# david-cortes/cmfrec

Measured on AMD Instinct MI355X. Metric: ALS rows/sec ((users+items)/iteration time), implicit ALS-CG k=50 fp64, higher is better.
Workload: dtype f64

## Files before the change

cmfrec_amd/csrc/cg_kernels.hpp:

```cpp
#pragma once
#include <hip/hip_runtime.h>
#include <stdint.h>
#include <type_traits>

#include "lanes.hpp"

namespace cmfhip {

constexpr int WAVE = 64;
constexpr int TILE = 64;
constexpr int MAX_W = 8;
#ifndef CMF_CG_WAVES_PER_SIMD
#define CMF_CG_WAVES_PER_SIMD 2
#endif
#ifndef CMF_CG_WAVES_PER_SIMD_F32
#define CMF_CG_WAVES_PER_SIMD_F32 3
#endif
#ifndef CMF_CG_WAVES_PER_SIMD_LOW
#define CMF_CG_WAVES_PER_SIMD_LOW 3
#endif
constexpr int CG_NTSEL_MAX_S = 7;
template <typename T, int W, int NRES_, int NTSEL = 0> constexpr int cg_waves_per_simd()
{
    if (sizeof(T) == 8 && NTSEL == 1 && W <= 8) return CMF_CG_WAVES_PER_SIMD_LOW;
    if (sizeof(T) == 4 && NTSEL == 1 && W <= 4 && NRES_ == 0) return CMF_CG_WAVES_PER_SIMD_F32 + 1;
    return (sizeof(T) == 4 && W <= 4 && NRES_ == 0) ? CMF_CG_WAVES_PER_SIMD_F32 : CMF_CG_WAVES_PER_SIMD;
}
constexpr int CG_NT_LOW = 6;
#ifndef CMF_CG_NT_F32
#define CMF_CG_NT_F32 1
#endif
#ifndef CMF_CG_NT_MIN_S
#define CMF_CG_NT_MIN_S 4
#endif

struct RowDesc {
    int row;
    int nnz;
    unsigned long long st;
};

constexpr int CG_NCOUNTERS = 64;
constexpr int CG_COUNTER_STRIDE = 32;

template <typename T>
__device__ __forceinline__ T cg_div(T num, T den)
{
#ifndef CMF_CG_IEEE_DIV
    if constexpr (sizeof(T) == 4) return num * __builtin_amdgcn_rcpf(den);
    else {
        double y = __builtin_amdgcn_rcp(den);
        double e = __builtin_fma(-den, y, 1.0);
        y = __builtin_fma(y, e, y);
        e = __builtin_fma(-den, y, 1.0);
        y = __builtin_fma(y, e, y);
        double q = num * y;
        const double r = __builtin_fma(-den, q, num);
        return __builtin_fma(r, y, q);
    }
#else
    return num / den;
#endif
}

template <typename V>
__device__ __forceinline__ V lds_g(const V *p) { return *p; }

template <typename T>
struct CgParams {
    T *A;
    size_t lda;
    const T *B;
    size_t ldb;
    int k;
    const size_t *indptr;
    const int *indices;
    const T *values;
    const T *bias_sub;
    const T *weights = nullptr;
    const T *wsum = nullptr;
    const int *order;
    const RowDesc *desc;
    int nrows;
    const T *BtB;
    T lam, lam_last;
    int scale_lam, scale_bias_const;
    int max_cg_steps;
    int precond;
    int koff = 0, kc = 0;
    const T *CtC = nullptr;
    const T *UC = nullptr;
    T w_side = 0;
    int rows_with_u = 0;
    int row_first = 0;
    const size_t *indptr2 = nullptr;
    const int *indices2 = nullptr;
    const T *values2 = nullptr;
    const T *C2 = nullptr;
    int *counter = nullptr;
    int p_side = 0, scale_lam_sideinfo = 0;
    const T *Bi = nullptr;
    const T *BiTBi = nullptr;
    int ki = 0;
    T w_imp = 0;
    const T *rconst = nullptr;
    size_t ldr = 0;
    int gx = 0;
#ifdef CMF_CG_DEBUG
    int dbg = 0;
#endif
#ifdef CMF_CG_TICKS
    unsigned long long *ticks = nullptr;
#endif
};
#ifdef CMF_CG_TICKS
#define CMF_TICK() __builtin_amdgcn_s_memtime()
__device__ __forceinline__ void cg_ticks_flush(unsigned long long *t, int slot, unsigned long long wait, unsigned long long pass, unsigned long long rows,
                                               unsigned long long total, int lane)
{
    if (t != nullptr && lane == 0) {
        atomicAdd(t + 4 * slot + 0, wait); atomicAdd(t + 4 * slot + 1, pass); atomicAdd(t + 4 * slot + 2, rows); atomicAdd(t + 4 * slot + 3, total);
    }
}
#endif
#ifdef CMF_CG_DEBUG
#define CMF_DBG(P, bit) (((P).dbg & (bit)) != 0)
#else
#define CMF_DBG(P, bit) false
#endif
template <int NT, int S, typename TILE, typename T>
__device__ __forceinline__ void dbg_fill_tile(TILE &tile, T val)
{
#pragma unroll
    for (int t = 0; t < NT; t++)
#pragma unroll
        for (int s = 0; s < S; s++) tile.set(t, s, val);
}

template <typename T>
__device__ __forceinline__ T wave_sum(T v) { return lanes::wave_sum(v); }

template <typename T, int NT, int I>
__device__ __forceinline__ T treduce8_low_first(const T (&v)[8], bool h)
{
    if constexpr (I + 4 < NT) {
        T keep = h ? v[I + 4] : v[I];
        return keep + lanes::recv_xor4(v[I], v[I + 4]);
    } else return v[I] + lanes::xor4_lower(v[I]);
}
template <typename T, int NT = 8>
__device__ __forceinline__ T treduce8_low(const T (&v)[8], int lane)
{
    static_assert(NT >= 4 && NT <= 8, "entries per lane group");
    T u[4], q[2];
    bool h = (lane & 4) != 0;
    u[0] = treduce8_low_first<T, NT, 0>(v, h); u[1] = treduce8_low_first<T, NT, 1>(v, h);
    u[2] = treduce8_low_first<T, NT, 2>(v, h); u[3] = treduce8_low_first<T, NT, 3>(v, h);
    h = (lane & 2) != 0;
#pragma unroll
    for (int i = 0; i < 2; i++) {
        T keep = h ? u[i + 2] : u[i];
        T send = h ? u[i] : u[i + 2];
        q[i] = keep + lanes::xor2(send);
    }
    h = (lane & 1) != 0;
    T keep = h ? q[1] : q[0];
    T send = h ? q[0] : q[1];
    return keep + lanes::xor1(send);
}

template <typename T>
__device__ __forceinline__ T treduce8_high(const T (&v)[8], int lane)
{
    T u[4], q[2];
#pragma unroll
    for (int i = 0; i < 4; i++) u[i] = lanes::tswap32_add(v[i], v[i + 4]);
#pragma unroll
    for (int i = 0; i < 2; i++) q[i] = lanes::tswap16_add(u[i], u[i + 2]);
    const bool h = (lane & 8) != 0;
    T keep = h ? q[1] : q[0];
    return keep + lanes::recv_xor8(q[0], q[1]);
}

#ifndef CMF_PASS_VECTOR_LDS
#define CMF_PASS_VECTOR_LDS 2
#endif
template <typename T> constexpr bool pass_vector_in_lds() { return CMF_PASS_VECTOR_LDS == 1 || (CMF_PASS_VECTOR_LDS == 2 && sizeof(T) == 8); }
template <typename T, int S>
__device__ __forceinline__ void replicate(T vdist, T (&vrep)[S], int lane);
template <typename T, int S, int GR = 8>
__device__ __forceinline__ void pass_vector_lds(T vdist, T (&vrep)[S], T (&wts)[8], int lane, T *__restrict__ pv)
{
    const int jj = lane >> 3, ll = lane & 7;
    pv[lane] = vdist;
    __builtin_amdgcn_wave_barrier();
#pragma unroll
    for (int s = 0; s < S; s++) vrep[s] = pv[ll + 8 * s];
    const T *wp = pv + GR * jj;
#pragma unroll
    for (int t = 0; t < GR; t++) wts[t] = wp[t];
    __builtin_amdgcn_wave_barrier();
}

__host__ __device__ constexpr int gram_ld(int S) { return 8 * S + 1; }
#ifndef CMF_GRAM_ROWS_BY_K
#define CMF_GRAM_ROWS_BY_K 1
#endif
template <typename T> __host__ __device__ constexpr int gram_rows(int S) { return (CMF_GRAM_ROWS_BY_K && pass_vector_in_lds<T>()) ? S : 8; }
__host__ __device__ constexpr int gram_ld_rows(int S, int GR)
{
    if (GR == 8) return gram_ld(S);
    int ld = 8 * S;
    while ((S * ld) % 32 != 8 && (S * ld) % 32 != 24) ld++;
    return ld;
}
__host__ __device__ constexpr int gram_ld2(int S) { return 8 * S + 2; }
template <typename T> __host__ __device__ constexpr int gram_elems(int S) { return sizeof(T) == 4 ? 64 * gram_ld2(S) : 64 * gram_ld(S); }
template <typename T, int S, int GR = 8> __device__ __forceinline__ int gram_index(int r, int c)
{
    if constexpr (sizeof(T) == 4) return 2 * ((r >> 1) * gram_ld2(S) + c) + (r & 1);
    else return r * gram_ld_rows(S, GR) + c;
}
template <typename T, int S, int GR = 8>
__device__ __forceinline__ void stage_gramian(T *__restrict__ G, const T *__restrict__ BtB, int k, int tid, int nthreads)
{
    static_assert(GR == 8 || sizeof(T) == 8, "rows by k: double precision");
    for (int e = tid; e < 8 * GR * 8 * S; e += nthreads) {
        const int r = e / (8 * S), c = e % (8 * S);
        G[gram_index<T, S, GR>(r, c)] = (r < k && c < k) ? BtB[(size_t)r * k + c] : T(0);
    }
}

template <typename T, int S>
struct RegTile {
    T v[8][S];
    __device__ __forceinline__ void set(int t, int s, T x) { v[t][s] = x; }
};
typedef float f32x2 __attribute__((ext_vector_type(2)));
template <int S>
struct RegTile<float, S> {
    f32x2 v[4][S];
    __device__ __forceinline__ void set(int t, int s, float x) { v[t >> 1][s][t & 1] = x; }
};

template <typename T>
struct PassAcc {
    T v[8];
    __device__ __forceinline__ void zero()
    {
#pragma unroll
        for (int s = 0; s < 8; s++) v[s] = T(0);
    }
    __device__ __forceinline__ void close(T (&out)[8]) const
    {
#pragma unroll
        for (int s = 0; s < 8; s++) out[s] = v[s];
    }
};
template <>
struct PassAcc<float> {
    f32x2 v[8];
    __device__ __forceinline__ void zero()
    {
#pragma unroll
        for (int s = 0; s < 8; s++) v[s] = f32x2{0.f, 0.f};
    }
    __device__ __forceinline__ void close(float (&out)[8]) const
    {
#pragma unroll
        for (int s = 0; s < 8; s++) out[s] = v[s][0] + v[s][1];
    }
};

template <typename T, int S, int NT = 8>
__device__ __forceinline__ void load_tile(RegTile<T, S> &tile, const T *__restrict__ Bm, size_t ldb,
                                          int k, int my_idx, int cnt, int lane)
{
    const int jj = lane >> 3, ll = lane & 7;
    int its[8];
    its[0] = lanes::bcast8<0>(my_idx); its[1] = lanes::bcast8<1>(my_idx); its[2] = lanes::bcast8<2>(my_idx);
    its[3] = lanes::bcast8<3>(my_idx);
    if (NT > 4) its[4] = lanes::bcast8<4>(my_idx);
    if (NT > 5) its[5] = lanes::bcast8<5>(my_idx);
    if (NT > 6) its[6] = lanes::bcast8<6>(my_idx);
    if (NT > 7) its[7] = lanes::bcast8<7>(my_idx);
    const int first_idx = __builtin_amdgcn_readfirstlane(my_idx);
    const int col_last = min(ll + 8 * (S - 1), k - 1) - ll;
    const char *base = reinterpret_cast<const char *>(Bm + ll);
    const unsigned ldb_bytes = (unsigned)(ldb * sizeof(T));
#pragma unroll
    for (int t = 0; t < NT; t++) {
        const unsigned it = (unsigned)(((jj * NT + t) < cnt) ? its[t] : first_idx);
        const T *rp = reinterpret_cast<const T *>(base + (unsigned long long)it * ldb_bytes);
#pragma unroll
        for (int s = 0; s < S; s++) tile.set(t, s, rp[(s < S - 1) ? 8 * s : col_last]);
    }
}

template <typename T, bool IMPLICIT, int MODE>
__device__ __forceinline__ T pass_weight(T coef, T x, bool valid, T g = T(1))
{
    T w;
    if (IMPLICIT) {
        if (MODE == 0) w = -(coef - T(1)) * x - coef;
        else           w = coef * (x - T(1)) + coef;
    } else {
        if (MODE == 0) w = -((coef - x) * g);
        else           w = coef * g;
    }
    return valid ? w : T(0);
}

template <typename T>
__device__ __forceinline__ T row_lam_mult(const CgParams<T> &P, int row, int nnz)
{
    return (P.wsum != nullptr) ? P.wsum[row] : (T)nnz;
}
template <typename T, bool IMPLICIT>
__device__ __forceinline__ T entry_weight(const CgParams<T> &P, size_t pos)
{
    if (IMPLICIT) return T(1);
    return (P.weights != nullptr) ? P.weights[pos] : T(1);
}

template <int S, bool IMPLICIT, int MODE, int NT = 8, bool INIT = false>
__device__ __forceinline__ void tile_pass_f32(const RegTile<float, S> &tile, const float (&vrep)[S], float x, bool valid,
                                          PassAcc<float> &out, int lane, float g = 1.f)
{
    static_assert(NT % 2 == 0, "single precision: the entries of a lane group travel in pairs");
    float c[8];
#pragma unroll
    for (int q = 0; q < NT / 2; q++) {
        f32x2 acc = f32x2{0.f, 0.f};
#pragma unroll
        for (int s = 0; s < S; s++) acc += tile.v[q][s] * f32x2{vrep[s], vrep[s]};
        c[2 * q] = acc[0]; c[2 * q + 1] = acc[1];
    }
    float coef = treduce8_low<float, NT>(c, lane);
    const float w = pass_weight<float, IMPLICIT, MODE>(coef, x, valid, g);
    float wts[8];
    wts[0] = lanes::bcast8<0>(w); wts[1] = lanes::bcast8<1>(w); wts[2] = lanes::bcast8<2>(w); wts[3] = lanes::bcast8<3>(w);
    if (NT > 4) { wts[4] = lanes::bcast8<4>(w); wts[5] = lanes::bcast8<5>(w); }
    if (NT > 6) { wts[6] = lanes::bcast8<6>(w); wts[7] = lanes::bcast8<7>(w); }
#pragma unroll
    for (int q = 0; q < NT / 2; q++) {
        const f32x2 w2 = f32x2{wts[2 * q], wts[2 * q + 1]};
#pragma unroll
        for (int s = 0; s < S; s++) out.v[s] = (INIT && q == 0) ? w2 * tile.v[q][s] : out.v[s] + w2 * tile.v[q][s];
    }
    if constexpr (INIT) {
#pragma unroll
        for (int s = S; s < 8; s++) out.v[s] = f32x2{0.f, 0.f};
    }
}

template <typename T, int S, bool IMPLICIT, int MODE, int NT = 8, bool INIT = false>
__device__ __forceinline__ void tile_pass(const RegTile<T, S> &tile, const T (&vrep)[S], T x, bool valid,
                                          PassAcc<T> &out, int lane, T g = T(1))
{
    if constexpr (std::is_same<T, float>::value) {
        tile_pass_f32<S, IMPLICIT, MODE, NT, INIT>(tile, vrep, x, valid, out, lane, g);
    } else {
    T c[8];
#pragma unroll
    for (int t = 0; t < NT; t++) {
        T acc = T(0);
#pragma unroll
        for (int s = 0; s < S; s++) acc += tile.v[t][s] * vrep[s];
        c[t] = acc;
    }
    T coef = treduce8_low<T, NT>(c, lane);
    const T w = pass_weight<T, IMPLICIT, MODE>(coef, x, valid, g);
    T wts[8];
    wts[0] = lanes::bcast8<0>(w); wts[1] = lanes::bcast8<1>(w); wts[2] = lanes::bcast8<2>(w); wts[3] = lanes::bcast8<3>(w);
    if (NT > 4) wts[4] = lanes::bcast8<4>(w);
    if (NT > 5) wts[5] = lanes::bcast8<5>(w);
    if (NT > 6) wts[6] = lanes::bcast8<6>(w);
    if (NT > 7) wts[7] = lanes::bcast8<7>(w);
#pragma unroll
    for (int t = 0; t < NT; t++) {
#pragma unroll
        for (int s = 0; s < S; s++) out.v[s] = (INIT && t == 0) ? wts[t] * tile.v[t][s] : out.v[s] + wts[t] * tile.v[t][s];
    }
    if constexpr (INIT) {
#pragma unroll
        for (int s = S; s < 8; s++) out.v[s] = T(0);
    }
    }
}

template <typename T, int S, int W>
__device__ __forceinline__ void gram_pass(const T *__restrict__ G, T wdist, PassAcc<T> &out, int lane, int wr)
{
    constexpr int LD = gram_ld(S);
    const int jj = lane >> 3, ll = lane & 7;
    T wts[8];
    wts[0] = lanes::bcast8<0>(wdist); wts[1] = lanes::bcast8<1>(wdist); wts[2] = lanes::bcast8<2>(wdist);
    wts[3] = lanes::bcast8<3>(wdist); wts[4] = lanes::bcast8<4>(wdist); wts[5] = lanes::bcast8<5>(wdist);
    wts[6] = lanes::bcast8<6>(wdist); wts[7] = lanes::bcast8<7>(wdist);
    if constexpr (std::is_same<T, float>::value && W <= 4) {
#pragma unroll
        for (int q = 0; q < 4; q++) {
            if (W > 1 && (q % W) != wr) continue;
            const f32x2 *g = reinterpret_cast<const f32x2 *>(G) + (jj * 4 + q) * gram_ld2(S) + ll;
            const f32x2 w2 = f32x2{wts[2 * q], wts[2 * q + 1]};
#pragma unroll
            for (int s = 0; s < S; s++) out.v[s] += w2 * lds_g(g + 8 * s);
        }
    } else {
#pragma unroll
        for (int t = 0; t < 8; t++) {
            if (W > 1 && (t % W) != wr) continue;
#pragma unroll
            for (int s = 0; s < S; s++) {
                if constexpr (std::is_same<T, float>::value) out.v[s][0] += wts[t] * G[gram_index<T, S>(jj * 8 + t, ll + 8 * s)];
                else out.v[s] += wts[t] * lds_g(G + (jj * 8 + t) * LD + ll + 8 * s);
            }
        }
    }
}

template <bool NEG, typename T, int S, int W, int GR = 8>
__device__ __forceinline__ void gram_pass_w(const T *__restrict__ G, const T (&wts)[8], PassAcc<T> &out, int lane, int wr)
{
    constexpr int LD = gram_ld_rows(S, GR);
    const int jj = lane >> 3, ll = lane & 7;
    if constexpr (std::is_same<T, float>::value && W <= 4) {
#pragma unroll
        for (int q = 0; q < 4; q++) {
            if (W > 1 && (q % W) != wr) continue;
            const f32x2 *g = reinterpret_cast<const f32x2 *>(G) + (jj * 4 + q) * gram_ld2(S) + ll;
            const f32x2 w2 = f32x2{wts[2 * q], wts[2 * q + 1]};
#pragma unroll
            for (int s = 0; s < S; s++) out.v[s] = NEG ? out.v[s] - w2 * lds_g(g + 8 * s) : out.v[s] + w2 * lds_g(g + 8 * s);
        }
    } else {
#pragma unroll
        for (int t = 0; t < GR; t++) {
            if (W > 1 && (t % W) != wr) continue;
#pragma unroll
            for (int s = 0; s < S; s++) {
                if constexpr (std::is_same<T, float>::value) {
                    const float g = G[gram_index<T, S>(jj * 8 + t, ll + 8 * s)];
                    out.v[s][0] = NEG ? out.v[s][0] - wts[t] * g : out.v[s][0] + wts[t] * g;
                } else {
                    const T g = lds_g(G + (jj * GR + t) * LD + ll + 8 * s);
                    out.v[s] = NEG ? out.v[s] - wts[t] * g : out.v[s] + wts[t] * g;
                }
            }
        }
    }
}

template <typename T, int S>
__device__ __forceinline__ void replicate(T vdist, T (&vrep)[S], int lane)
{
    const int ll = lane & 7;
#pragma unroll
    for (int s = 0; s < S; s++) vrep[s] = __shfl(vdist, s * 8 + ll);
}

template <typename T, int S, bool IMPLICIT, int W, int RPB, bool GRAMX = false, int NRES_ = 0, int NTSEL = 0>
__global__ void __launch_bounds__(64 * W * RPB, (cg_waves_per_simd<T, W, NRES_, NTSEL>()))
cg_rows_kernel(const CgParams<T> P)
{
    constexpr bool GRAM = IMPLICIT || GRAMX;
    extern __shared__ __attribute__((aligned(16))) unsigned char smem_raw[];
    T *G = reinterpret_cast<T *>(smem_raw);
    T *red = G + (GRAM ? gram_elems<T>(S) : 0);
    const int tid = threadIdx.x;
    const int lane = tid & 63;
    const int wave = tid >> 6;
    const int grp = wave / W;
    const int wr = wave % W;
    const int k = P.k;

    const int nteams = gridDim.x * RPB;
    __shared__ int s_claim[4];
    constexpr bool PV = pass_vector_in_lds<T>();
    __shared__ __attribute__((aligned(16))) T s_pv[PV ? W * RPB : 1][PV ? 64 : 1];
    const int cslot = (blockIdx.x * RPB + grp) % CG_NCOUNTERS;
    int *const my_counter = P.counter + cslot * CG_COUNTER_STRIDE;
    const int cbase = nteams + cslot;
    auto issue_claim = [&]() -> int {
        int v = 0;
        if (wr == 0 && lane == 0) v = atomicAdd(my_counter, 1);
        return v;
    };
    int rnxt, rnn;
    if (W == 1) {
        const int c1 = issue_claim(), c2 = issue_claim();
        rnxt = cbase + CG_NCOUNTERS * __builtin_amdgcn_readfirstlane(c1);
        rnn = cbase + CG_NCOUNTERS * __builtin_amdgcn_readfirstlane(c2);
    } else if (wr == 0 && lane == 0) {
        s_claim[2] = cbase + CG_NCOUNTERS * atomicAdd(my_counter, 1);
        s_claim[3] = cbase + CG_NCOUNTERS * atomicAdd(my_counter, 1);
    }
    constexpr int GR = gram_rows<T>(S);
    if (GRAM) stage_gramian<T, S, GR>(G, P.BtB, k, tid, blockDim.x);
    if (GRAM || W > 1) __syncthreads();
    if (W > 1) { rnxt = s_claim[2]; rnn = s_claim[3]; }
    T *myred = red + (size_t)grp * 2 * W * 64;

    int buf = 0;
    static_assert(W == 1 || RPB == 1, "multi-wave teams own their workgroup (barriers are per row)");

    constexpr int NRES = NRES_ > 0 ? NRES_ : ((std::is_same<T, float>::value && W == 8) ? 2 : 1);
    static_assert(NRES == 1 || std::is_same<T, float>::value, "two resident tiles: single precision");
    static_assert(NTSEL == 0 || (S >= CMF_CG_NT_MIN_S && (sizeof(T) == 4 || S <= CG_NTSEL_MAX_S) && NRES_ == 0),
                  "launches by tile size: tiles by row length (double precision: k <= 56)");
    constexpr int NT_MIN = (S >= CMF_CG_NT_MIN_S && (CMF_CG_NT_F32 || !std::is_same<T, float>::value)) ? (std::is_same<T, float>::value ? 6 : 5) : 8;
    auto nt_of = [&](int nnz_) -> int {
        int nt = (nnz_ + 8 * W * NRES - 1) / (8 * W * NRES);
        if (std::is_same<T, float>::value) nt = (nt + 1) & ~1;
        return (nt > 8) ? 8 : (nt < NT_MIN ? NT_MIN : nt);
    };
    struct Pre { int idx; T x; T a; int idx2; T x2; T g; T g2; };
    auto load_desc = [&](int rix_) -> RowDesc {
        RowDesc d; d.row = 0; d.nnz = 0; d.st = 0;
        if (rix_ < P.nrows) d = P.desc[rix_];
        d.row = __builtin_amdgcn_readfirstlane(d.row);
        d.nnz = __builtin_amdgcn_readfirstlane(d.nnz);
        d.st = ((unsigned long long)(unsigned)__builtin_amdgcn_readfirstlane((int)(d.st >> 32)) << 32) |
               (unsigned)__builtin_amdgcn_readfirstlane((int)(d.st & 0xffffffffu));
        return d;
    };
    auto load_pre = [&](const RowDesc &d) -> Pre {
        Pre q; q.idx = 0; q.x = T(0); q.a = T(0); q.idx2 = 0; q.x2 = T(0); q.g = T(1); q.g2 = T(1);
        const int nt = nt_of(d.nnz), tl = 8 * nt;
        const int b = lane & 7;
        const int ent = (lane >> 3) * nt + b;
        const int cnt = min(tl, d.nnz - wr * tl);
        if (b < nt && ent < cnt) {
            const size_t pos = d.st + (size_t)wr * tl + ent;
            q.idx = P.indices[pos];
            q.x = P.values[pos];
            q.g = entry_weight<T, IMPLICIT>(P, pos);
            if (!IMPLICIT && P.bias_sub != nullptr) q.x -= P.bias_sub[q.idx];
        }
        if (NRES == 2) {
            const int cnt2 = min(tl, d.nnz - (wr + W) * tl);
            if (b < nt && ent < cnt2) {
                const size_t pos = d.st + (size_t)(wr + W) * tl + ent;
                q.idx2 = P.indices[pos];
                q.x2 = P.values[pos];
                q.g2 = entry_weight<T, IMPLICIT>(P, pos);
                if (!IMPLICIT && P.bias_sub != nullptr) q.x2 -= P.bias_sub[q.idx2];
            }
        }
        if (d.nnz > 0 && lane < k) q.a = P.A[(size_t)d.row * P.lda + lane];
        return q;
    };
    int rix = blockIdx.x * RPB + grp;
    RowDesc dcur = load_desc(rix);
    RowDesc dnxt = load_desc(rnxt);
    Pre pcur = load_pre(dcur);
    int pend = issue_claim();
#ifdef CMF_CG_TICKS
    unsigned long long tk_wait = 0, tk_pass = 0, tk_rows = 0;
    const unsigned long long tk_begin = CMF_TICK();
#endif
    int it = 0;
    RowDesc dnn;
    Pre pnxt;
    auto solve_row = [&](auto nt_tag) {
        constexpr int NT = decltype(nt_tag)::value;
        constexpr int TL = 8 * NT;
        const int row = dcur.row;
        const size_t st = dcur.st;
        const int nnz = dcur.nnz;
        const int ntiles = (nnz + TL - 1) / TL;
        const int my_ntiles = (ntiles > wr) ? (ntiles - wr + W - 1) / W : 0;
        const bool resident = NT < 8 || my_ntiles <= NRES;

        T lam = P.lam, lam_last = P.lam_last;
        if (GRAMX && P.kc > 0) {
            if (P.scale_lam || P.scale_lam_sideinfo) {
                T mult = row_lam_mult(P, row, nnz);
                if (P.scale_lam_sideinfo) mult += (T)P.p_side;
                lam *= mult; lam_last *= mult;
            }
        } else if (!IMPLICIT && P.scale_lam) {
            const T mult = row_lam_mult(P, row, nnz);
            lam *= mult;
            if (!P.scale_bias_const) lam_last *= mult;
        }
        T *arow = P.A + (size_t)row * P.lda;
        T a_d = pcur.a;

        RegTile<T, S> tile;
        const int ent = (lane >> 3) * NT + (lane & 7);
        const bool lane_has = (NT == 8) || (lane & 7) < NT;
        const int cnt0 = min(TL, nnz - wr * TL);
        T x_res = pcur.x;
        const T g_res = pcur.g;
        bool valid_res = lane_has && ent < cnt0;
        if (CMF_DBG(P, 1)) dbg_fill_tile<8, S>(tile, (T)(pcur.idx & 3) * (T)0.001);
        else if (cnt0 > 0) load_tile<T, S, NT>(tile, P.B, P.ldb, k, pcur.idx, cnt0, lane);
        RegTile<T, (NRES == 2) ? S : 1> tile2;
        const int cnt1 = (NRES == 2) ? min(TL, nnz - (wr + W) * TL) : 0;
        const T x2_res = pcur.x2, g2_res = pcur.g2;
        const bool valid2_res = lane_has && ent < cnt1;
        if constexpr (NRES == 2) {
            if (cnt1 > 0 && !CMF_DBG(P, 1)) load_tile<T, S, NT>(tile2, P.B, P.ldb, k, pcur.idx2, cnt1, lane);
        }
        dnn = load_desc(rnn);
        pnxt = load_pre(dnxt);
#ifdef CMF_CG_TICKS
        const unsigned long long tk0 = CMF_TICK();
        asm volatile("s_waitcnt vmcnt(0)" ::: "memory");
        const unsigned long long tk1 = CMF_TICK();
        tk_wait += tk1 - tk0;
#endif

        auto run_pass = [&](T vdist, auto mode_tag, bool first) -> T {
            constexpr int MODE = decltype(mode_tag)::value;
            asm volatile("" ::: "memory");
            T vrep[S];
            T gw[8];
            if constexpr (PV) pass_vector_lds<T, S, GR>(vdist, vrep, gw, lane, &s_pv[wave][0]);
            else replicate<T, S>(vdist, vrep, lane);
            PassAcc<T> acc;
            acc.zero();
            if constexpr (NRES == 2) {
                if (cnt0 > 0 && !CMF_DBG(P, 4)) tile_pass<T, S, IMPLICIT, MODE, NT>(tile, vrep, x_res, valid_res, acc, lane, g_res);
                if (cnt1 > 0 && !CMF_DBG(P, 4)) tile_pass<T, S, IMPLICIT, MODE, NT>(tile2, vrep, x2_res, valid2_res, acc, lane, g2_res);
            } else if constexpr (NT < 8) {
                if (cnt0 > 0 && !CMF_DBG(P, 4)) tile_pass<T, S, IMPLICIT, MODE, NT>(tile, vrep, x_res, valid_res, acc, lane, g_res);
            } else
            for (int tl = wr; tl < ntiles; tl += W) {
                T x, g; bool valid;
                const bool have = (tl == wr) && (resident || first);
                if (!have) {
                    const int cnt = min(TL, nnz - tl * TL);
                    valid = lane_has && ent < cnt;
                    const size_t pos = st + (size_t)tl * TL + ent;
                    int my_idx = valid ? P.indices[pos] : 0;
                    x = valid ? P.values[pos] : T(0);
                    g = valid ? entry_weight<T, IMPLICIT>(P, pos) : T(1);
                    if (!IMPLICIT && P.bias_sub != nullptr && valid) x -= P.bias_sub[my_idx];
                    if (!CMF_DBG(P, 1)) load_tile<T, S, NT>(tile, P.B, P.ldb, k, my_idx, cnt, lane);
                } else {
                    x = x_res; g = g_res; valid = valid_res;
                }
                if (!CMF_DBG(P, 4)) tile_pass<T, S, IMPLICIT, MODE, NT>(tile, vrep, x, valid, acc, lane, g);
            }
            if (GRAM && !CMF_DBG(P, 2)) {
                if constexpr (PV) gram_pass_w<MODE == 0, T, S, W, GR>(G, gw, acc, lane, wr);
                else gram_pass<T, S, W>(G, (MODE == 0) ? -vdist : vdist, acc, lane, wr);
            }
            T out[8];
            acc.close(out);
            T tot = treduce8_high<T>(out, lane);
            if (W > 1) {
                T *rb = myred + (size_t)buf * W * 64;
                rb[wr * 64 + lane] = tot;
                if (first && wr == 0 && lane == 0) s_claim[it & 1] = cbase + CG_NCOUNTERS * pend;
                __syncthreads();
                tot = T(0);
#pragma unroll
                for (int w = 0; w < W; w++) tot += rb[w * 64 + lane];
                buf ^= 1;
            }
            return tot;
        };

        T r_d = run_pass(a_d, std::integral_constant<int, 0>{}, true);
        r_d -= lam * a_d;
        if (!IMPLICIT && lam != lam_last && lane == k - 1) r_d -= (lam_last - lam) * a_d;
        if (GRAMX && P.rconst != nullptr && lane < k) r_d += P.rconst[(size_t)row * P.ldr + lane];
        if (lane >= k) r_d = T(0);
        T p_d = r_d;
        T r_old = CMF_DBG(P, 8) ? T(1) : wave_sum(r_d * r_d);
        bool done = (r_old <= (T)1e-12);
        for (int step = 0; step < P.max_cg_steps && !done; step++) {
            T Ap_d = run_pass(p_d, std::integral_constant<int, 1>{}, false);
            Ap_d += lam * p_d;
            if (!IMPLICIT && lam != lam_last && lane == k - 1) Ap_d += (lam_last - lam) * p_d;
            if (lane >= k) Ap_d = T(0);
            T alpha = CMF_DBG(P, 8) ? T(0.001) : cg_div(r_old, wave_sum(Ap_d * p_d));
            a_d += alpha * p_d;
            r_d -= alpha * Ap_d;
            T r_new = CMF_DBG(P, 8) ? T(0.5) : wave_sum(r_d * r_d);
            if (r_new <= (T)1e-8) done = true;
            else {
                p_d = p_d * cg_div(r_new, r_old) + r_d;
                r_old = r_new;
            }
        }
        if (wr == 0 && lane < k) arow[lane] = a_d;
#ifdef CMF_CG_TICKS
        tk_pass += CMF_TICK() - tk1; tk_rows += (wr == 0);
#endif
    };
    for (; rix < P.nrows; it++) {
        const int nt = nt_of(dcur.nnz);
        if constexpr (NT_MIN == 8) solve_row(std::integral_constant<int, 8>{});
        else if constexpr (std::is_same<T, float>::value) {
            if constexpr (NTSEL == 1) solve_row(std::integral_constant<int, 6>{});
            else if constexpr (NTSEL == 2) solve_row(std::integral_constant<int, 8>{});
            else if (nt == 6) solve_row(std::integral_constant<int, 6>{});
            else solve_row(std::integral_constant<int, 8>{});
        } else if constexpr (NTSEL == 1) {
            if (nt <= 5) solve_row(std::integral_constant<int, 5>{});
            else solve_row(std::integral_constant<int, 6>{});
        } else if constexpr (NTSEL == 2) {
            if (nt <= 7) solve_row(std::integral_constant<int, 7>{});
            else solve_row(std::integral_constant<int, 8>{});
        } else {
            switch (nt) {
                case 5: solve_row(std::integral_constant<int, 5>{}); break;
                case 6: solve_row(std::integral_constant<int, 6>{}); break;
                case 7: solve_row(std::integral_constant<int, 7>{}); break;
                default: solve_row(std::integral_constant<int, 8>{}); break;
            }
        }
        const int r3 = (W == 1) ? cbase + CG_NCOUNTERS * __builtin_amdgcn_readfirstlane(pend) : s_claim[it & 1];
        dcur = dnxt; dnxt = dnn; pcur = pnxt;
        rix = rnxt; rnxt = rnn; rnn = r3;
        pend = issue_claim();
    }
#ifdef CMF_CG_TICKS
    cg_ticks_flush(P.ticks, W == 1 ? 0 : W == 2 ? 1 : W == 4 ? 2 : 3, tk_wait, tk_pass, tk_rows, CMF_TICK() - tk_begin, lane);
#endif
}

constexpr int TILE4 = 32;

template <typename T, int S>
struct RegTile4 {
    T v[4][S];
    __device__ __forceinline__ void set(int t, int s, T x) { v[t][s] = x; }
    __device__ __forceinline__ T get(int t, int s) const { return v[t][s]; }
};
template <int S>
struct RegTile4<float, S> {
    f32x2 v[2][S];
    __device__ __forceinline__ void set(int t, int s, float x) { v[t >> 1][s][t & 1] = x; }
    __device__ __forceinline__ f32x2 pair0(int s) const { return v[0][s]; }
};

template <typename T, int S>
__device__ __forceinline__ void load_tile4(RegTile4<T, S> &tile, const T *__restrict__ Bm, size_t ldb,
                                           int k, int my_idx, int cnt, int lane)
{
    const int jj = lane >> 3, ll = lane & 7;
    int its[4];
    its[0] = lanes::bcast8<0>(my_idx); its[1] = lanes::bcast8<2>(my_idx);
    its[2] = lanes::bcast8<4>(my_idx); its[3] = lanes::bcast8<6>(my_idx);
    const int first_idx = __builtin_amdgcn_readfirstlane(my_idx);
    const int col_last = min(ll + 8 * (S - 1), k - 1) - ll;
    const char *base = reinterpret_cast<const char *>(Bm + ll);
    const unsigned ldb_bytes = (unsigned)(ldb * sizeof(T));
#pragma unroll
    for (int t = 0; t < 4; t++) {
        const unsigned it = (unsigned)(((jj * 4 + t) < cnt) ? its[t] : first_idx);
        const T *rp = reinterpret_cast<const T *>(base + (unsigned long long)it * ldb_bytes);
#pragma unroll
        for (int s = 0; s < S; s++) tile.set(t, s, rp[(s < S - 1) ? 8 * s : col_last]);
    }
}

template <typename T>
__device__ __forceinline__ T treduce4_low(const T (&v)[4], int lane)
{
    T u[2];
    bool h = (lane & 4) != 0;
#pragma unroll
    for (int i = 0; i < 2; i++) {
        T keep = h ? v[i + 2] : v[i];
        u[i] = keep + lanes::recv_xor4(v[i], v[i + 2]);
    }
    h = (lane & 2) != 0;
    T keep = h ? u[1] : u[0];
    T send = h ? u[0] : u[1];
    T q = keep + lanes::xor2(send);
    return q + lanes::xor1(q);
}

template <int S, bool IMPLICIT, int MODE, typename TILE, bool INIT = false>
__device__ __forceinline__ void tile_pass4_f32(const TILE &tile, const float (&vrep)[S], float x, bool valid,
                                           PassAcc<float> &out, int lane, float g = 1.f)
{
    float c[4];
#pragma unroll
    for (int q = 0; q < 2; q++) {
        f32x2 acc = f32x2{0.f, 0.f};
#pragma unroll
        for (int s = 0; s < S; s++) acc += tile.v[q][s] * f32x2{vrep[s], vrep[s]};
        c[2 * q] = acc[0]; c[2 * q + 1] = acc[1];
    }
    float coef = treduce4_low<float>(c, lane);
    const float w = pass_weight<float, IMPLICIT, MODE>(coef, x, valid, g);
    float wts[4];
    wts[0] = lanes::bcast8<0>(w); wts[1] = lanes::bcast8<2>(w); wts[2] = lanes::bcast8<4>(w); wts[3] = lanes::bcast8<6>(w);
#pragma unroll
    for (int q = 0; q < 2; q++) {
        const f32x2 w2 = f32x2{wts[2 * q], wts[2 * q + 1]};
#pragma unroll
        for (int s = 0; s < S; s++) out.v[s] = (INIT && q == 0) ? w2 * tile.v[q][s] : out.v[s] + w2 * tile.v[q][s];
    }
    if constexpr (INIT) {
#pragma unroll
        for (int s = S; s < 8; s++) out.v[s] = f32x2{0.f, 0.f};
    }
}

template <typename T, int S, bool IMPLICIT, int MODE, typename TILE, bool INIT = false>
__device__ __forceinline__ void tile_pass4(const TILE &tile, const T (&vrep)[S], T x, bool valid,
                                           PassAcc<T> &out, int lane, T g = T(1))
{
    if constexpr (std::is_same<T, float>::value) {
        tile_pass4_f32<S, IMPLICIT, MODE, TILE, INIT>(tile, vrep, x, valid, out, lane, g);
    } else {
    T c[4];
#pragma unroll
    for (int t = 0; t < 4; t++) {
        T acc = T(0);
#pragma unroll
        for (int s = 0; s < S; s++) acc += tile.v[t][s] * vrep[s];
        c[t] = acc;
    }
    T coef = treduce4_low<T>(c, lane);
    const T w = pass_weight<T, IMPLICIT, MODE>(coef, x, valid, g);
    T wts[4];
    wts[0] = lanes::bcast8<0>(w); wts[1] = lanes::bcast8<2>(w); wts[2] = lanes::bcast8<4>(w); wts[3] = lanes::bcast8<6>(w);
#pragma unroll
    for (int t = 0; t < 4; t++) {
#pragma unroll
        for (int s = 0; s < S; s++) out.v[s] = (INIT && t == 0) ? wts[t] * tile.v[t][s] : out.v[s] + wts[t] * tile.v[t][s];
    }
    if constexpr (INIT) {
#pragma unroll
        for (int s = S; s < 8; s++) out.v[s] = T(0);
    }
    }
}

template <typename T, int S>
struct RegTile2 {
    T v[2][S];
    __device__ __forceinline__ void set(int t, int s, T x) { v[t][s] = x; }
    __device__ __forceinline__ T get(int t, int s) const { return v[t][s]; }
};
template <int S>
struct RegTile2<float, S> {
    f32x2 v[S];
    __device__ __forceinline__ void set(int t, int s, float x) { v[s][t] = x; }
    __device__ __forceinline__ f32x2 pair0(int s) const { return v[s]; }
};

template <typename T, int S, typename TILE>
__device__ __forceinline__ void load_tile2(TILE &tile, const T *__restrict__ Bm, size_t ldb,
                                           int k, int my_idx, int cnt, int lane)
{
    const int jj = lane >> 3, ll = lane & 7;
    int its[2];
    its[0] = lanes::bcast8<0>(my_idx); its[1] = lanes::bcast8<4>(my_idx);
    const int first_idx = __builtin_amdgcn_readfirstlane(my_idx);
    const int col_last = min(ll + 8 * (S - 1), k - 1) - ll;
    const char *base = reinterpret_cast<const char *>(Bm + ll);
    const unsigned ldb_bytes = (unsigned)(ldb * sizeof(T));
#pragma unroll
    for (int t = 0; t < 2; t++) {
        const unsigned it = (unsigned)(((jj * 2 + t) < cnt) ? its[t] : first_idx);
        const T *rp = reinterpret_cast<const T *>(base + (unsigned long long)it * ldb_bytes);
#pragma unroll
        for (int s = 0; s < S; s++) tile.set(t, s, rp[(s < S - 1) ? 8 * s : col_last]);
    }
}

template <typename T>
__device__ __forceinline__ T treduce2_low(const T (&v)[2], int lane)
{
    const bool h = (lane & 4) != 0;
    T u = (h ? v[1] : v[0]) + lanes::recv_xor4(v[0], v[1]);
    u += lanes::xor2(u);
    return u + lanes::xor1(u);
}

template <typename T, int S, bool IMPLICIT, int MODE, typename TILE, bool INIT = false>
__device__ __forceinline__ void tile_pass2(const TILE &tile, const T (&vrep)[S], T x, bool valid,
                                           PassAcc<T> &out, int lane, T g = T(1))
{
    T c[2];
    if constexpr (std::is_same<T, float>::value) {
        f32x2 acc = f32x2{0.f, 0.f};
#pragma unroll
        for (int s = 0; s < S; s++) acc += tile.pair0(s) * f32x2{vrep[s], vrep[s]};
        c[0] = acc[0]; c[1] = acc[1];
    } else {
#pragma unroll
        for (int t = 0; t < 2; t++) {
            T acc = T(0);
#pragma unroll
            for (int s = 0; s < S; s++) acc += tile.get(t, s) * vrep[s];
            c[t] = acc;
        }
    }
    const T coef = treduce2_low<T>(c, lane);
    const T w = pass_weight<T, IMPLICIT, MODE>(coef, x, valid, g);
    const T w0 = lanes::bcast8<0>(w), w1 = lanes::bcast8<4>(w);
    if constexpr (std::is_same<T, float>::value) {
        const f32x2 w2 = f32x2{w0, w1};
#pragma unroll
        for (int s = 0; s < S; s++) out.v[s] = INIT ? w2 * tile.pair0(s) : out.v[s] + w2 * tile.pair0(s);
        if constexpr (INIT) {
#pragma unroll
            for (int s = S; s < 8; s++) out.v[s] = f32x2{0.f, 0.f};
        }
    } else {
#pragma unroll
        for (int s = 0; s < S; s++) out.v[s] = INIT ? w0 * tile.get(0, s) : out.v[s] + w0 * tile.get(0, s);
#pragma unroll
        for (int s = 0; s < S; s++) out.v[s] += w1 * tile.get(1, s);
        if constexpr (INIT) {
#pragma unroll
            for (int s = S; s < 8; s++) out.v[s] = T(0);
        }
    }
}

template <typename T, int S, int NE> struct TinyTile { using type = RegTile4<T, S>; };
template <typename T, int S> struct TinyTile<T, S, 2> { using type = RegTile2<T, S>; };

#ifndef CMF_TINY_WAVES_PER_SIMD
#define CMF_TINY_WAVES_PER_SIMD 4
#endif
#ifndef CMF_TINY_GREG_F32
#define CMF_TINY_GREG_F32 1
#endif
#ifndef CMF_TINY_GREG_F64
#define CMF_TINY_GREG_F64 1
#endif
template <typename T, bool GRAM> constexpr bool tiny_greg() { return GRAM && (sizeof(T) == 8 ? CMF_TINY_GREG_F64 != 0 : CMF_TINY_GREG_F32 != 0); }
template <typename T, bool GRAM> constexpr int tiny_waves_per_simd() { return tiny_greg<T, GRAM>() ? (sizeof(T) == 8 ? 2 : 3) : CMF_TINY_WAVES_PER_SIMD; }
template <typename T, int S, int GR = 8>
struct GramRegs {
    T v[GR][S];
    __device__ __forceinline__ void load(const T *__restrict__ G, int lane)
    {
        const int jj = lane >> 3, ll = lane & 7;
#pragma unroll
        for (int t = 0; t < GR; t++)
#pragma unroll
            for (int s = 0; s < S; s++) v[t][s] = G[gram_index<T, S, GR>(jj * GR + t, ll + 8 * s)];
    }
};
template <int S>
struct GramRegs<float, S, 8> {
    f32x2 v[4][S];
    __device__ __forceinline__ void load(const float *__restrict__ G, int lane)
    {
        const int jj = lane >> 3, ll = lane & 7;
#pragma unroll
        for (int q = 0; q < 4; q++) {
            const f32x2 *g = reinterpret_cast<const f32x2 *>(G) + (jj * 4 + q) * gram_ld2(S) + ll;
#pragma unroll
            for (int s = 0; s < S; s++) v[q][s] = g[8 * s];
        }
    }
};
template <int S>
__device__ __forceinline__ void gram_pass_regs(const GramRegs<float, S> &R, float wdist, PassAcc<float> &out)
{
    float wts[8];
    wts[0] = lanes::bcast8<0>(wdist); wts[1] = lanes::bcast8<1>(wdist); wts[2] = lanes::bcast8<2>(wdist);
    wts[3] = lanes::bcast8<3>(wdist); wts[4] = lanes::bcast8<4>(wdist); wts[5] = lanes::bcast8<5>(wdist);
    wts[6] = lanes::bcast8<6>(wdist); wts[7] = lanes::bcast8<7>(wdist);
#pragma unroll
    for (int q = 0; q < 4; q++) {
        const f32x2 w2 = f32x2{wts[2 * q], wts[2 * q + 1]};
#pragma unroll
        for (int s = 0; s < S; s++) out.v[s] += w2 * R.v[q][s];
    }
}
template <typename T, int S>
__device__ __forceinline__ void gram_pass_regs(const GramRegs<T, S> &R, T wdist, PassAcc<T> &out)
{
    T wts[8];
    wts[0] = lanes::bcast8<0>(wdist); wts[1] = lanes::bcast8<1>(wdist); wts[2] = lanes::bcast8<2>(wdist);
    wts[3] = lanes::bcast8<3>(wdist); wts[4] = lanes::bcast8<4>(wdist); wts[5] = lanes::bcast8<5>(wdist);
    wts[6] = lanes::bcast8<6>(wdist); wts[7] = lanes::bcast8<7>(wdist);
#pragma unroll
    for (int t = 0; t < 8; t++)
#pragma unroll
        for (int s = 0; s < S; s++) out.v[s] += wts[t] * R.v[t][s];
}

template <bool NEG, int S>
__device__ __forceinline__ void gram_pass_regs_w(const GramRegs<float, S> &R, const float (&wts)[8], PassAcc<float> &out)
{
#pragma unroll
    for (int q = 0; q < 4; q++) {
        const f32x2 w2 = f32x2{wts[2 * q], wts[2 * q + 1]};
#pragma unroll
        for (int s = 0; s < S; s++) out.v[s] = NEG ? out.v[s] - w2 * R.v[q][s] : out.v[s] + w2 * R.v[q][s];
    }
}
template <bool NEG, typename T, int S, int GR>
__device__ __forceinline__ void gram_pass_regs_w(const GramRegs<T, S, GR> &R, const T (&wts)[8], PassAcc<T> &out)
{
#pragma unroll
    for (int t = 0; t < GR; t++)
#pragma unroll
        for (int s = 0; s < S; s++) out.v[s] = NEG ? out.v[s] - wts[t] * R.v[t][s] : out.v[s] + wts[t] * R.v[t][s];
}

template <typename T, int S, bool IMPLICIT, bool GRAMX = false, int NE = 4>
__global__ void __launch_bounds__(256, (tiny_waves_per_simd<T, IMPLICIT || GRAMX>()))
cg_rows_tiny_kernel(const CgParams<T> P)
{
    static_assert(NE == 4 || NE == 2 || NE == 0, "entries per lane group");
    constexpr bool MIX = NE == 0;
    static_assert(!MIX || CMF_TINY_WAVES_PER_SIMD >= 3, "the mixed launch lives in the dynamically scheduled loop");
    using Tile = typename TinyTile<T, S, (NE == 2) ? 2 : 4>::type;
    constexpr bool GRAM = IMPLICIT || GRAMX;
    extern __shared__ __attribute__((aligned(16))) unsigned char smem_raw[];
    T *G = reinterpret_cast<T *>(smem_raw);
    constexpr bool PV = pass_vector_in_lds<T>();
    __shared__ __attribute__((aligned(16))) T s_pv[PV ? 4 : 1][PV ? 64 : 1];
    const int tid = threadIdx.x;
    const int lane = tid & 63;
    auto short_row = [&](int nnz_) -> bool { return MIX && nnz_ <= 16; };
    auto entry_of = [&](int nnz_) -> int { return (NE == 2 || short_row(nnz_)) ? (lane >> 2) : (lane >> 1); };
    const int k = P.k;
    constexpr bool GREG = tiny_greg<T, GRAM>();
    constexpr int GR = GREG ? gram_rows<T>(S) : 8;
    if (GRAM) {
        stage_gramian<T, S, GR>(G, P.BtB, k, tid, blockDim.x);
        __syncthreads();
    }
    GramRegs<T, GREG ? S : 1, GREG ? GR : 8> greg;
    if constexpr (GREG) greg.load(G, lane);
    const int nwaves = gridDim.x * 4;
    struct Pre { int idx; T x; T a; T g; };
    auto load_desc = [&](int rix_) -> RowDesc {
        RowDesc d; d.row = 0; d.nnz = 0; d.st = 0;
        if (rix_ < P.nrows) d = P.desc[rix_];
        d.row = __builtin_amdgcn_readfirstlane(d.row);
        d.nnz = __builtin_amdgcn_readfirstlane(d.nnz);
        d.st = ((unsigned long long)(unsigned)__builtin_amdgcn_readfirstlane((int)(d.st >> 32)) << 32) |
               (unsigned)__builtin_amdgcn_readfirstlane((int)(d.st & 0xffffffffu));
        return d;
    };
    auto load_pre = [&](const RowDesc &d) -> Pre {
        Pre q; q.idx = 0; q.x = T(0); q.a = T(0); q.g = T(1);
        const int ent = entry_of(d.nnz);
        if (ent < d.nnz) {
            const size_t pos = d.st + (size_t)ent;
            q.idx = P.indices[pos];
            q.x = P.values[pos];
            q.g = entry_weight<T, IMPLICIT>(P, pos);
            if (!IMPLICIT && P.bias_sub != nullptr) q.x -= P.bias_sub[q.idx];
        }
        if (d.nnz > 0 && lane < k) q.a = P.A[(size_t)d.row * P.lda + lane];
        return q;
    };
    auto load_tile_ne = [&](Tile &t_, const T *Bm_, size_t ldb_, int k_, int idx_, int cnt_, int lane_) {
        if constexpr (NE != 2) load_tile4<T, S>(t_, Bm_, ldb_, k_, idx_, cnt_, lane_);
        else load_tile2<T, S>(t_, Bm_, ldb_, k_, idx_, cnt_, lane_);
    };
    auto solve = [&](const RowDesc &d, const Pre &pr, const Tile &tile, auto short_tag) {
        constexpr bool T2 = NE == 2 || decltype(short_tag)::value;
        const int nnz = d.nnz;
        T lam = P.lam, lam_last = P.lam_last;
        if (GRAMX && P.kc > 0) {
            if (P.scale_lam || P.scale_lam_sideinfo) {
                T mult = row_lam_mult(P, d.row, nnz);
                if (P.scale_lam_sideinfo) mult += (T)P.p_side;
                lam *= mult; lam_last *= mult;
            }
        } else if (!IMPLICIT && P.scale_lam) {
            const T mult = row_lam_mult(P, d.row, nnz);
            lam *= mult;
            if (!P.scale_bias_const) lam_last *= mult;
        }
        const bool valid = (T2 ? (lane >> 2) : (lane >> 1)) < nnz;
        T a_d = pr.a;
        auto run_pass = [&](T vdist, auto mode_tag) -> T {
            constexpr int MODE = decltype(mode_tag)::value;
            asm volatile("" ::: "memory");
            T vrep[S];
            T gw[8];
            if constexpr (PV) pass_vector_lds<T, S, GR>(vdist, vrep, gw, lane, &s_pv[tid >> 6][0]);
            else replicate<T, S>(vdist, vrep, lane);
            PassAcc<T> acc;
            if (!CMF_DBG(P, 4)) {
                if constexpr (!T2) tile_pass4<T, S, IMPLICIT, MODE, decltype(tile), true>(tile, vrep, pr.x, valid, acc, lane, pr.g);
                else tile_pass2<T, S, IMPLICIT, MODE, decltype(tile), true>(tile, vrep, pr.x, valid, acc, lane, pr.g);
            } else acc.zero();
            if constexpr (GREG) {
                if (!CMF_DBG(P, 2)) {
                    if constexpr (PV) gram_pass_regs_w<MODE == 0>(greg, gw, acc);
                    else gram_pass_regs(greg, (MODE == 0) ? -vdist : vdist, acc);
                }
            }
            else if (GRAM && !CMF_DBG(P, 2)) gram_pass<T, S, 1>(G, (MODE == 0) ? -vdist : vdist, acc, lane, 0);
            T out[8];
            acc.close(out);
            return treduce8_high<T>(out, lane);
        };
        T r_d = run_pass(a_d, std::integral_constant<int, 0>{});
        r_d -= lam * a_d;
        if (!IMPLICIT && lam != lam_last && lane == k - 1) r_d -= (lam_last - lam) * a_d;
        if (GRAMX && P.rconst != nullptr && lane < k) r_d += P.rconst[(size_t)d.row * P.ldr + lane];
        if (lane >= k) r_d = T(0);
        T p_d = r_d;
        T r_old = wave_sum(r_d * r_d);
        bool done = (r_old <= (T)1e-12);
        for (int step = 0; step < P.max_cg_steps && !done; step++) {
            T Ap_d = run_pass(p_d, std::integral_constant<int, 1>{});
            Ap_d += lam * p_d;
            if (!IMPLICIT && lam != lam_last && lane == k - 1) Ap_d += (lam_last - lam) * p_d;
            if (lane >= k) Ap_d = T(0);
            T alpha = cg_div(r_old, wave_sum(Ap_d * p_d));
            a_d += alpha * p_d;
            r_d -= alpha * Ap_d;
            T r_new = wave_sum(r_d * r_d);
            if (r_new <= (T)1e-8) done = true;
            else {
                p_d = p_d * cg_div(r_new, r_old) + r_d;
                r_old = r_new;
            }
        }
        if (lane < k) P.A[(size_t)d.row * P.lda + lane] = a_d;
    };

    int rix = blockIdx.x * 4 + (tid >> 6);
#if CMF_TINY_WAVES_PER_SIMD >= 3
    {
        const int cslot = rix % CG_NCOUNTERS;
        int *const my_counter = P.counter + cslot * CG_COUNTER_STRIDE;
        const int cbase = nwaves + cslot;
        auto issue_claim = [&]() -> int {
            int v = 0;
            if (lane == 0) v = atomicAdd(my_counter, 1);
            return v;
        };
        const int c1 = issue_claim(), c2 = issue_claim();
        int rnxt = cbase + CG_NCOUNTERS * __builtin_amdgcn_readfirstlane(c1);
        int rnn = cbase + CG_NCOUNTERS * __builtin_amdgcn_readfirstlane(c2);
        RowDesc d0 = load_desc(rix), d1 = load_desc(rnxt);
        Pre p0 = load_pre(d0);
        Tile tA;
        int pend = issue_claim();
        while (rix < P.nrows) {
            const bool shrt = short_row(d0.nnz);
            if (CMF_DBG(P, 1)) {
                dbg_fill_tile<(NE == 2) ? 2 : 4, S>(tA, (T)(p0.idx & 3) * (T)0.001);
            } else if constexpr (MIX) {
                if (shrt) load_tile2<T, S>(tA, P.B, P.ldb, k, p0.idx, d0.nnz, lane);
                else load_tile_ne(tA, P.B, P.ldb, k, p0.idx, d0.nnz, lane);
            } else load_tile_ne(tA, P.B, P.ldb, k, p0.idx, d0.nnz, lane);
            RowDesc d2 = load_desc(rnn);
            Pre p1 = load_pre(d1);
            if constexpr (MIX) {
                if (shrt) solve(d0, p0, tA, std::true_type{});
                else solve(d0, p0, tA, std::false_type{});
            } else solve(d0, p0, tA, std::false_type{});
            const int r3 = cbase + CG_NCOUNTERS * __builtin_amdgcn_readfirstlane(pend);
            d0 = d1; p0 = p1; d1 = d2;
            rix = rnxt; rnxt = rnn; rnn = r3;
            pend = issue_claim();
        }
        return;
    }
#endif
    RowDesc d0 = load_desc(rix), d1 = load_desc(rix + nwaves), d2 = load_desc(rix + 2 * nwaves);
    Pre p0 = load_pre(d0);
    Tile tA, tB;
    if (d0.nnz > 0) load_tile_ne(tA, P.B, P.ldb, k, p0.idx, d0.nnz, lane);
    Pre p1 = load_pre(d1);
    while (rix < P.nrows) {
        if (d1.nnz > 0) load_tile_ne(tB, P.B, P.ldb, k, p1.idx, d1.nnz, lane);
        RowDesc d3 = load_desc(rix + 3 * nwaves);
        Pre p2 = load_pre(d2);
        solve(d0, p0, tA, std::false_type{});
        rix += nwaves;
        if (rix >= P.nrows) break;
        if (d2.nnz > 0) load_tile_ne(tA, P.B, P.ldb, k, p2.idx, d2.nnz, lane);
        RowDesc d4 = load_desc(rix + 3 * nwaves);
        Pre p3 = load_pre(d3);
        solve(d1, p1, tB, std::false_type{});
        rix += nwaves;
        d0 = d2; p0 = p2; d1 = d3; p1 = p3; d2 = d4;
    }
}

constexpr int VH_CHUNK_TILES = 4;

struct VhWork {
    int vi;
    int row;
    int cnt;
    int chunk;
    unsigned long long st;
    unsigned long long pad_;
};

template <typename T>
struct VhState {
    T *r, *p;
    T *r_old;
    int *done;
    T *part;
    const int *chunk_row;
    const int *chunk_start;
    const int *chunk_cnt;
    const int *chunk_off;
    const int *launch;
    const VhWork *work;
    int nvh, nchunks, nlaunch;
};

template <typename T, int S, bool IMPLICIT, int MODE>
__global__ void __launch_bounds__(64 * VH_CHUNK_TILES, 3)
vh_pass_kernel(const CgParams<T> P, const VhState<T> V)
{
    __shared__ T red[VH_CHUNK_TILES][64];
    const int lane = threadIdx.x & 63, wave = threadIdx.x >> 6;
    const VhWork wk = V.work[blockIdx.x];
    const int vi = wk.vi;
    if (vi < 0) return;
    if (MODE == 1 && V.done[vi]) return;
    const int c = wk.chunk;
    const int row = wk.row;
    const size_t st = (size_t)wk.st;
    const int nnz = wk.cnt;
    const int tl = wave;
    const int k = P.k;
    T vdist;
    if (MODE == 0) vdist = (lane < k) ? P.A[(size_t)row * P.lda + lane] : T(0);
    else           vdist = V.p[(size_t)vi * 64 + lane];
    PassAcc<T> acc;
    acc.zero();
    if (tl * TILE < nnz) {
        const int cnt = min(TILE, nnz - tl * TILE);
        const bool valid = lane < cnt;
        const size_t pos = st + (size_t)tl * TILE + lane;
        int my_idx = valid ? P.indices[pos] : 0;
        T x = valid ? P.values[pos] : T(0);
        const T g = valid ? entry_weight<T, IMPLICIT>(P, pos) : T(1);
        if (!IMPLICIT && P.bias_sub != nullptr && valid) x -= P.bias_sub[my_idx];
        RegTile<T, S> tile;
        if (CMF_DBG(P, 1)) dbg_fill_tile<8, S>(tile, (T)(my_idx & 3) * (T)0.001);
        else load_tile<T, S>(tile, P.B, P.ldb, k, my_idx, cnt, lane);
        T vrep[S];
        replicate<T, S>(vdist, vrep, lane);
        if (!CMF_DBG(P, 4)) tile_pass<T, S, IMPLICIT, MODE>(tile, vrep, x, valid, acc, lane, g);
    }
    T out[8];
    acc.close(out);
    T tot = treduce8_high<T>(out, lane);
    red[wave][lane] = tot;
    __syncthreads();
    if (wave == 0) {
        T s = T(0);
#pragma unroll
        for (int w = 0; w < VH_CHUNK_TILES; w++) s += red[w][lane];
        V.part[(size_t)c * 64 + lane] = s;
    }
}

constexpr int VH_UPD_WAVES = 4;

template <typename T, bool IMPLICIT, int MODE, bool GRAMX = false>
__global__ void __launch_bounds__(64 * VH_UPD_WAVES)
vh_update_kernel(const CgParams<T> P, const VhState<T> V)
{
    __shared__ T psum[VH_UPD_WAVES][64];
    const int lane = threadIdx.x & 63, wave = threadIdx.x >> 6;
    const int vi = blockIdx.x;
    if (MODE == 1 && V.done[vi]) return;
    const int k = P.k;
    const int row = P.order[vi];
    const int nnz = (int)(P.indptr[row + 1] - P.indptr[row]);
    {
        const int c0 = V.chunk_off[vi], c1 = V.chunk_off[vi + 1];
        T acc = T(0);
        int c = c0 + wave;
        for (; c + 3 * VH_UPD_WAVES < c1; c += 4 * VH_UPD_WAVES) {
            T v0 = V.part[(size_t)c * 64 + lane];
            T v1 = V.part[(size_t)(c + VH_UPD_WAVES) * 64 + lane];
            T v2 = V.part[(size_t)(c + 2 * VH_UPD_WAVES) * 64 + lane];
            T v3 = V.part[(size_t)(c + 3 * VH_UPD_WAVES) * 64 + lane];
            acc += v0; acc += v1; acc += v2; acc += v3;
        }
        for (; c < c1; c += VH_UPD_WAVES) acc += V.part[(size_t)c * 64 + lane];
        psum[wave][lane] = acc;
    }
    __syncthreads();
    if (wave != 0) return;
    T tot = T(0);
#pragma unroll
    for (int w = 0; w < VH_UPD_WAVES; w++) tot += psum[w][lane];
    T lam = P.lam, lam_last = P.lam_last;
    if (GRAMX && P.kc > 0) {
        if (P.scale_lam || P.scale_lam_sideinfo) {
            T mult = row_lam_mult(P, row, nnz);
            if (P.scale_lam_sideinfo) mult += (T)P.p_side;
            lam *= mult; lam_last *= mult;
        }
    } else if (!IMPLICIT && P.scale_lam) {
        const T mult = row_lam_mult(P, row, nnz);
        lam *= mult;
        if (!P.scale_bias_const) lam_last *= mult;
    }
    T *arow = P.A + (size_t)row * P.lda;
    T a_d = (lane < k) ? arow[lane] : T(0);
    T v = (MODE == 0) ? a_d : V.p[(size_t)vi * 64 + lane];
    if (IMPLICIT || GRAMX) {
        T g = T(0);
        for (int j = 0; j < k; j++) {
            T vj = __shfl(v, j);
            if (lane < k) g += vj * P.BtB[(size_t)j * k + lane];
        }
        tot += (MODE == 0) ? -g : g;
    }
    if (MODE == 0) {
        T r_d = tot - lam * a_d;
        if (!IMPLICIT && lam != lam_last && lane == k - 1) r_d -= (lam_last - lam) * a_d;
        if (GRAMX && P.rconst != nullptr && lane < k) r_d += P.rconst[(size_t)row * P.ldr + lane];
        if (lane >= k) r_d = T(0);
        T r_old = wave_sum(r_d * r_d);
        V.r[(size_t)vi * 64 + lane] = r_d;
        V.p[(size_t)vi * 64 + lane] = r_d;
        if (lane == 0) { V.r_old[vi] = r_old; V.done[vi] = (r_old <= (T)1e-12) ? 1 : 0; }
    } else {
        T p_d = v;
        T r_d = V.r[(size_t)vi * 64 + lane];
        T r_old = V.r_old[vi];
        T Ap_d = tot + lam * p_d;
        if (!IMPLICIT && lam != lam_last && lane == k - 1) Ap_d += (lam_last - lam) * p_d;
        if (lane >= k) Ap_d = T(0);
        T alpha = cg_div(r_old, wave_sum(Ap_d * p_d));
        a_d += alpha * p_d;
        r_d -= alpha * Ap_d;
        T r_new = wave_sum(r_d * r_d);
        if (lane < k) arow[lane] = a_d;
        if (r_new <= (T)1e-8) {
            if (lane == 0) V.done[vi] = 1;
        } else {
            V.p[(size_t)vi * 64 + lane] = p_d * cg_div(r_new, r_old) + r_d;
            V.r[(size_t)vi * 64 + lane] = r_d;
            if (lane == 0) V.r_old[vi] = r_new;
        }
    }
}

template <typename T, int NF, bool IMPLICIT, int TEAM>
__global__ void __launch_bounds__(TEAM == 16 ? 1024 : 256)
cg_rows_generic_kernel(const CgParams<T> P)
{
    static_assert(TEAM == 1 || TEAM == 4 || TEAM == 16, "team");
    __shared__ T red[TEAM][64 * NF];
    const int lane = threadIdx.x & 63, wv = threadIdx.x >> 6;
    const int unit_global = (TEAM == 1) ? ((blockIdx.x * blockDim.x + threadIdx.x) >> 6) : (int)blockIdx.x;
    const int nunits = (TEAM == 1) ? ((gridDim.x * blockDim.x) >> 6) : (int)gridDim.x;
    const int kx = P.k, koff = P.koff, kt = koff + kx, kc = P.kc;
    const bool coll = kc > 0;
    for (int rix = P.row_first + unit_global; rix < P.nrows; rix += nunits) {
        const int row = P.order[rix];
        const size_t st = P.indptr[row];
        const int nnz = (int)(P.indptr[row + 1] - st);
        const bool has_u = coll && row < P.rows_with_u;
        if (!IMPLICIT && nnz == 0 && !has_u && P.gx == 1 && P.Bi != nullptr) {
            if (TEAM == 1 || wv == 0)
                for (int f = lane; f < kt; f += 64) P.A[(size_t)row * P.lda + f] = T(0);
            continue;
        }
        if (nnz == 0 && !has_u && !(P.gx != 0 && !IMPLICIT)) {
            if (P.Bi != nullptr && (TEAM == 1 || wv == 0))
                for (int f = lane; f < kt; f += 64) P.A[(size_t)row * P.lda + f] = T(0);
            continue;
        }
        const bool sparse_u = P.indptr2 != nullptr;
        const size_t st2 = (sparse_u && has_u) ? P.indptr2[row] : 0;
        const int nnz2 = (sparse_u && has_u) ? (int)(P.indptr2[row + 1] - st2) : 0;
        if (sparse_u && has_u && nnz == 0 && nnz2 == 0 && P.gx != 2) {
            if (TEAM == 1 || wv == 0)
                for (int f = lane; f < kt; f += 64) P.A[(size_t)row * P.lda + f] = T(0);
            continue;
        }
        const int lo = (has_u || (!IMPLICIT && P.Bi != nullptr)) ? 0 : koff;
        T lam = P.lam, lam_last = P.lam_last;
        if (!IMPLICIT) {
            if (has_u) {
                if (P.scale_lam || P.scale_lam_sideinfo) {
                    T mult = (P.wsum != nullptr) ? P.wsum[row] : ((nnz > 0) ? (T)nnz : T(1));
                    if (P.scale_lam_sideinfo) mult += sparse_u ? (T)nnz2 : (T)P.p_side;
                    lam *= mult; lam_last *= mult;
                }
            } else if (P.scale_lam) {
                const T mult = row_lam_mult(P, row, nnz);
                lam *= mult;
                if (!P.scale_bias_const) lam_last *= mult;
            }
        }
        T *arow = P.A + (size_t)row * P.lda;
        const T *ucrow = (has_u && !sparse_u) ? P.UC + (size_t)row * kc : nullptr;
        T a[NF], r[NF], p[NF], Ap[NF];
#pragma unroll
        for (int c = 0; c < NF; c++) { int f = lane + 64 * c; a[c] = (f >= lo && f < kt) ? arow[f] : T(0); }

        auto bcast = [&](const T (&v)[NF], int j) {
            T vj = T(0);
#pragma unroll
            for (int c = 0; c < NF; c++) if (c == (j >> 6)) vj = __shfl(v[c], j & 63);
            return vj;
        };
        auto matvec = [&](const T (&v)[NF], T (&out)[NF], int mode) {
#pragma unroll
            for (int c = 0; c < NF; c++) out[c] = T(0);
            if (IMPLICIT || P.gx != 0) {
                for (int j = 0; j < kx; j++) {
                    T vj = bcast(v, koff + j);
                    if (mode == 0) vj = -vj;
#pragma unroll
                    for (int c = 0; c < NF; c++) { int f = lane + 64 * c; if (f >= koff && f < kt) out[c] += vj * P.BtB[(size_t)j * kx + (f - koff)]; }
                }
            }
            if (has_u && !sparse_u) {
                T acc[NF];
#pragma unroll
                for (int c = 0; c < NF; c++) acc[c] = T(0);
                for (int j = 0; j < kc; j++) {
                    const T vj = bcast(v, j);
#pragma unroll
                    for (int c = 0; c < NF; c++) { int f = lane + 64 * c; if (f < kc) acc[c] += vj * P.CtC[(size_t)j * kc + f]; }
                }
#pragma unroll
                for (int c = 0; c < NF; c++) {
                    int f = lane + 64 * c;
                    if (f < kc) out[c] += (mode == 0) ? P.w_side * (ucrow[f] - acc[c]) : P.w_side * acc[c];
                }
            }
            if (!IMPLICIT && P.Bi != nullptr) {
                T acc[NF];
#pragma unroll
                for (int c = 0; c < NF; c++) acc[c] = T(0);
                for (int j0 = 0; j0 < P.ki; j0 += 4) {
                    T mrow[4][NF];
#pragma unroll
                    for (int u = 0; u < 4; u++) {
                        const int j = min(j0 + u, P.ki - 1);
#pragma unroll
                        for (int c = 0; c < NF; c++) {
                            int f = lane + 64 * c;
                            mrow[u][c] = (f >= koff && f < koff + P.ki) ? P.BiTBi[(size_t)j * P.ki + (f - koff)] : T(0);
                        }
                    }
#pragma unroll
                    for (int u = 0; u < 4; u++) {
                        if (j0 + u >= P.ki) break;
                        const T vj = bcast(v, koff + j0 + u);
#pragma unroll
                        for (int c = 0; c < NF; c++) acc[c] += vj * mrow[u][c];
                    }
                }
#pragma unroll
                for (int c = 0; c < NF; c++) out[c] += (mode == 0) ? -P.w_imp * acc[c] : P.w_imp * acc[c];
            }
            T gat[NF];
#pragma unroll
            for (int c = 0; c < NF; c++) gat[c] = T(0);
            constexpr int UNR = 4;
            for (int j0 = (TEAM == 1 ? 0 : wv); j0 < nnz; j0 += TEAM * UNR) {
                int idx[UNR]; T x[UNR]; T gw[UNR]; T bv[UNR][NF]; T part[UNR];
#pragma unroll
                for (int u = 0; u < UNR; u++) {
                    const int j = j0 + u * TEAM;
                    const bool ok = j < nnz;
                    idx[u] = ok ? P.indices[st + j] : 0;
                    x[u] = ok ? P.values[st + j] : T(0);
                    gw[u] = ok ? entry_weight<T, IMPLICIT>(P, st + j) : T(1);
                }
#pragma unroll
                for (int u = 0; u < UNR; u++) {
                    const bool ok = (j0 + u * TEAM) < nnz;
                    if (!IMPLICIT && P.bias_sub != nullptr && ok) x[u] -= P.bias_sub[idx[u]];
                    const T *b = P.B + (size_t)idx[u] * P.ldb;
                    part[u] = T(0);
#pragma unroll
                    for (int c = 0; c < NF; c++) { int f = lane + 64 * c; bv[u][c] = (ok && f >= koff && f < kt) ? b[f - koff] : T(0); part[u] += bv[u][c] * v[c]; }
                }
#pragma unroll
                for (int u = 0; u < UNR; u++) part[u] = wave_sum(part[u]);
#pragma unroll
                for (int u = 0; u < UNR; u++) {
                    if ((j0 + u * TEAM) >= nnz) break;
                    const T coef = part[u];
                    T w;
                    if (IMPLICIT) w = (mode == 0) ? (-(coef - T(1)) * x[u] - coef) : (coef * (x[u] - T(1)) + coef);
                    else          w = (mode == 0) ? -((coef - x[u]) * gw[u]) : coef * gw[u];
#pragma unroll
                    for (int c = 0; c < NF; c++) gat[c] += w * bv[u][c];
                    if (!IMPLICIT && mode == 0 && P.Bi != nullptr) {
                        const T *bi = P.Bi + (size_t)idx[u] * P.ki;
#pragma unroll
                        for (int c = 0; c < NF; c++) { int f = lane + 64 * c; if (f >= koff && f < koff + P.ki) gat[c] += P.w_imp * bi[f - koff]; }
                    }
                }
            }
            for (int j = (TEAM == 1 ? 0 : wv); j < nnz2; j += TEAM) {
                const T *cj = P.C2 + (size_t)P.indices2[st2 + j] * kc;
                const T uj = P.values2[st2 + j];
                T cv[NF]; T part = T(0);
#pragma unroll
                for (int c = 0; c < NF; c++) { int f = lane + 64 * c; cv[c] = (f < kc) ? cj[f] : T(0); part += cv[c] * v[c]; }
                const T coef = wave_sum(part);
                const T w = (mode == 0) ? P.w_side * (-coef + uj) : P.w_side * coef;
#pragma unroll
                for (int c = 0; c < NF; c++) gat[c] += w * cv[c];
            }
            if (TEAM > 1) {
                __syncthreads();
#pragma unroll
                for (int c = 0; c < NF; c++) red[wv][lane + 64 * c] = gat[c];
                __syncthreads();
#pragma unroll
                for (int c = 0; c < NF; c++) {
                    T sacc = T(0);
#pragma unroll
                    for (int w2 = 0; w2 < TEAM; w2++) sacc += red[w2][lane + 64 * c];
                    gat[c] = sacc;
                }
            }
#pragma unroll
            for (int c = 0; c < NF; c++) out[c] += gat[c];
        };
        auto vdot = [&](const T (&u)[NF], const T (&v)[NF]) {
            T s = T(0);
#pragma unroll
            for (int c = 0; c < NF; c++) s += u[c] * v[c];
            return wave_sum(s);
        };
        auto live = [&](int f) { return f >= lo && f < kt; };
        matvec(a, r, 0);
#pragma unroll
        for (int c = 0; c < NF; c++) {
            int f = lane + 64 * c;
            r[c] -= lam * a[c];
            if (!IMPLICIT && lam != lam_last && f == kt - 1) r[c] -= (lam_last - lam) * a[c];
            if (!IMPLICIT && P.gx != 0 && P.rconst != nullptr && f >= koff && f < kt) r[c] += P.rconst[(size_t)row * P.ldr + (f - koff)];
            if (!live(f)) r[c] = T(0);
            p[c] = r[c];
        }
        if (P.precond) {
            T PC[NF], z[NF];
#pragma unroll
            for (int c = 0; c < NF; c++) PC[c] = T(0);
            for (int j = (TEAM == 1 ? 0 : wv); j < nnz; j += TEAM) {
                const int idx = P.indices[st + j];
                T x = P.values[st + j];
                const T gwt = entry_weight<T, IMPLICIT>(P, st + j);
                const T *b = P.B + (size_t)idx * P.ldb;
#pragma unroll
                for (int c = 0; c < NF; c++) {
                    int f = lane + 64 * c;
                    T bv = (f >= koff && f < kt) ? b[f - koff] : T(0);
                    PC[c] += IMPLICIT ? x * (bv * bv) : gwt * (bv * bv);
                }
            }
            for (int j = (TEAM == 1 ? 0 : wv); j < nnz2; j += TEAM) {
                const T *cj = P.C2 + (size_t)P.indices2[st2 + j] * kc;
#pragma unroll
                for (int c = 0; c < NF; c++) {
                    int f = lane + 64 * c;
                    T cvv = (f < kc) ? cj[f] : T(0);
                    PC[c] += cvv * cvv;
                }
            }
            if (TEAM > 1) {
                __syncthreads();
#pragma unroll
                for (int c = 0; c < NF; c++) red[wv][lane + 64 * c] = PC[c];
                __syncthreads();
#pragma unroll
                for (int c = 0; c < NF; c++) {
                    T sacc = T(0);
#pragma unroll
                    for (int w2 = 0; w2 < TEAM; w2++) sacc += red[w2][lane + 64 * c];
                    PC[c] = sacc;
                }
            }
#pragma unroll
            for (int c = 0; c < NF; c++) {
                int f = lane + 64 * c;
                if (has_u && !sparse_u && f < kc) PC[c] += P.CtC[(size_t)f * kc + f];
                if (!IMPLICIT && P.Bi != nullptr && f >= koff && f < koff + P.ki)
                    PC[c] += P.BiTBi[(size_t)(f - koff) * P.ki + (f - koff)];
                if (IMPLICIT) PC[c] += (f >= koff && f < kt) ? P.BtB[(size_t)(f - koff) * kx + (f - koff)] : T(0);
                else {
                    if (P.gx != 0) PC[c] += (f >= koff && f < kt) ? P.BtB[(size_t)(f - koff) * kx + (f - koff)] : T(0);
                    PC[c] += lam;
                    if (lam != lam_last && f == kt - 1) PC[c] += (lam_last - lam);
                }
                PC[c] = live(f) ? T(1) / PC[c] : T(0);
                z[c] = r[c] * PC[c];
                p[c] = z[c];
            }
            T r_old = vdot(z, r);
            for (int step = 0; step < P.max_cg_steps; step++) {
                matvec(p, Ap, 1);
#pragma unroll
                for (int c = 0; c < NF; c++) {
                    int f = lane + 64 * c;
                    Ap[c] += lam * p[c];
                    if (!IMPLICIT && lam != lam_last && f == kt - 1) Ap[c] += (lam_last - lam) * p[c];
                    if (!live(f)) Ap[c] = T(0);
                }
                T alpha = cg_div(r_old, vdot(Ap, p));
#pragma unroll
                for (int c = 0; c < NF; c++) {
                    a[c] += alpha * p[c]; r[c] -= alpha * Ap[c];
                    z[c] = r[c] * PC[c];
                }
                T r_new = vdot(z, r);
                T ratio = cg_div(r_new, r_old);
#pragma unroll
                for (int c = 0; c < NF; c++) p[c] = p[c] * ratio + z[c];
                r_old = r_new;
            }
        } else {
        T r_old = vdot(r, r);
        if (r_old > (T)1e-12) {
            for (int step = 0; step < P.max_cg_steps; step++) {
                matvec(p, Ap, 1);
#pragma unroll
                for (int c = 0; c < NF; c++) {
                    int f = lane + 64 * c;
                    Ap[c] += lam * p[c];
                    if (!IMPLICIT && lam != lam_last && f == kt - 1) Ap[c] += (lam_last - lam) * p[c];
                    if (!live(f)) Ap[c] = T(0);
                }
                T alpha = cg_div(r_old, vdot(Ap, p));
#pragma unroll
                for (int c = 0; c < NF; c++) { a[c] += alpha * p[c]; r[c] -= alpha * Ap[c]; }
                T r_new = vdot(r, r);
                if (r_new <= (T)1e-8) break;
                T ratio = cg_div(r_new, r_old);
#pragma unroll
                for (int c = 0; c < NF; c++) p[c] = p[c] * ratio + r[c];
                r_old = r_new;
            }
        }
        }
        if (TEAM == 1 || wv == 0) {
#pragma unroll
            for (int c = 0; c < NF; c++) { int f = lane + 64 * c; if (live(f)) arow[f] = a[c]; }
        }
    }
}

}
```

cmfrec_amd/csrc/device.hpp:

```cpp
#pragma once
#include <hip/hip_runtime.h>
#include <algorithm>
#include <cstdio>
#include <cstdlib>
#include <cstring>
#include <numeric>
#include <string>
#include <vector>

#include "../../include/cmfrec_hip.h"
#include "device_base.hpp"
#include "cg_kernels.hpp"
#include "chol_kernels.hpp"
#include "dense_kernels.hpp"
#include "gram_cg_kernels.hpp"
#include "topn_kernels.hpp"

namespace cmfhip {

constexpr int MAX_DEVICES = 16;
constexpr int NBINS = 6;
constexpr int BIN_VHEAVY = 0;
constexpr int BIN_HEAVY = 1;
constexpr int BIN_MED4 = 2;
constexpr int BIN_MED2 = 3;
constexpr int BIN_LIGHT = 4;
constexpr int BIN_TINY = 5;
constexpr int BIN_MIN_NNZ[NBINS] = {1025, 257, 129, 65, 33, 1};
inline int vh_min_env()
{
    const int v = switches().vh_min;
    return v > 0 ? std::min(sizeof(real_t) == 4 ? BIN_MIN_NNZ[BIN_VHEAVY] : (1 << 30), std::max(258, v)) : 0;
}

struct SparseShard {
    int nrows = 0;
    size_t nnz = 0;
    int vh_min = BIN_MIN_NNZ[BIN_VHEAVY];
    size_t opp_row_bytes_hint = 50 * sizeof(real_t);
    int bin_of(long long l) const
    {
        if (l >= vh_min) return BIN_VHEAVY;
        for (int b = 1; b < NBINS; b++)
            if (l >= BIN_MIN_NNZ[b]) return b;
        return -1;
    }
    static bool gram_pays(double vh_nnz, int n_other_, size_t opp_bytes_per_row)
    {
        (void)vh_nnz; (void)opp_bytes_per_row;
        return sizeof(real_t) == 4 || n_other_ > 0;
    }
    DevBuf<size_t> p;
    DevBuf<int> i;
    DevBuf<real_t> v;
    DevBuf<real_t> w, wsum;
    DevBuf<real_t> wsum_naz;
    bool weighted() const { return w.ptr != nullptr && nnz > 0; }
    DevBuf<int> order;
    DevBuf<RowDesc> desc;
    int bin_rows[NBINS] = {0, 0, 0, 0, 0, 0};
    int bin_first[NBINS] = {0, 0, 0, 0, 0, 0};
    size_t bin_nnz[NBINS] = {0, 0, 0, 0, 0, 0};
    int n_nonempty = 0, n_empty = 0;
    int max_nnz = 0;
    int n_long = 0;
    int n_gt96 = 0;
    int n_gt16 = 0;
    int n_gt512 = 0;
    int n_gt_low[4] = {0, 0, 0, 0};
    bool is_part = false;
    int n_other = 0;
    bool prefer_gram(size_t opp_bytes_per_row) const { return gram_pays((double)bin_nnz[0], n_other, opp_bytes_per_row); }
    bool vh_runs_aside(int num_cus) const
    {
        return bin_rows[0] > 0 && n_chunks <= 4 * num_cus;
    }
    static constexpr int LONG_ROW = 1024;
    int rows_longer_than(int maxlen, int cap) const
    {
        int n;
        if (maxlen >= max_nnz) n = 0;
        else if (maxlen >= LONG_ROW) n = n_long;
        else if (maxlen >= 256) n = bin_first[BIN_MED4];
        else if (maxlen >= 128) n = bin_first[BIN_MED2];
        else if (maxlen >= 96) n = n_gt96;
        else if (maxlen >= 64) n = bin_first[BIN_LIGHT];
        else if (maxlen >= 32) n = bin_first[BIN_TINY];
        else n = n_nonempty;
        return std::min(n, cap);
    }
    int n_chunks = 0;
    DevBuf<int> vh_chunk_row, vh_chunk_start, vh_chunk_cnt, vh_chunk_off, vh_launch, vh_done;
    DevBuf<VhWork> vh_work;
    int n_launch = 0;
    DevBuf<real_t> vh_r, vh_p, vh_r_old, vh_part;
    static constexpr int GRAM_SLICE = 2048;
    int slice_len = GRAM_SLICE;
    int n_slices = 0;
    DevBuf<int> sl_vrow, sl_first, sl_count, row_sl_off;
    std::vector<int> h_row_sl_off;
    DevBuf<real_t> gram_part;
    mutable DevBuf<real_t> chol_part;

    void upload(int nrows_, const size_t *hp, const int *hi, const real_t *hv, hipStream_t st, const real_t *hw = nullptr)
    {
        nrows = nrows_;
        nnz = hp[nrows] - hp[0];
        std::vector<size_t> p0(nrows + 1);
        for (int r = 0; r <= nrows; r++) p0[r] = hp[r] - hp[0];
        p.upload(p0.data(), nrows + 1, st);
        i.upload(hi + hp[0], nnz, st);
        v.upload(hv + hp[0], nnz, st);
        w.release(); wsum.release();
        if (hw != nullptr && nnz > 0) {
            w.upload(hw + hp[0], nnz, st);
            std::vector<real_t> ws((size_t)nrows);
            for (int r = 0; r < nrows; r++) {
                double acc_w = 0;
                for (size_t e = hp[r]; e < hp[r + 1]; e++) acc_w += hw[e];
                ws[r] = (hp[r + 1] > hp[r]) ? (real_t)acc_w : (real_t)1;
            }
            wsum.upload(ws.data(), (size_t)nrows, st);
            HIP_CHECK(hipStreamSynchronize(st));
        }
        std::vector<int> ord(nrows);
        std::iota(ord.begin(), ord.end(), 0);
        auto len = [&](int r) { return (long long)(p0[r + 1] - p0[r]); };
        std::stable_sort(ord.begin(), ord.end(), [&](int a, int b) { return len(a) > len(b); });
        std::vector<RowDesc> dsc(nrows);
        std::vector<unsigned> lens(nrows);
        for (int q = 0; q < nrows; q++) {
            const int r = ord[q];
            dsc[q].row = r; dsc[q].nnz = (int)len(r); dsc[q].st = (unsigned long long)p0[r];
            lens[q] = (unsigned)len(r);
        }
        order.upload(ord.data(), nrows, st);
        desc.upload(dsc.data(), nrows, st);
        build_bins(lens.data(), st);
        HIP_CHECK(hipStreamSynchronize(st));
    }

    void set_vh_chunks(const std::vector<int> &c_row, const std::vector<int> &c_start, const std::vector<int> &c_cnt,
                       const std::vector<int> &c_off, std::vector<int> launch, hipStream_t st)
    {
        n_chunks = (int)c_row.size();
        if (launch.empty()) { launch.resize(n_chunks); std::iota(launch.begin(), launch.end(), 0); }
        n_launch = (int)launch.size();
        vh_chunk_row.upload(c_row.data(), c_row.size(), st);
        vh_chunk_start.upload(c_start.data(), c_start.size(), st);
        vh_chunk_cnt.upload(c_cnt.data(), c_cnt.size(), st);
        vh_chunk_off.upload(c_off.data(), c_off.size(), st);
        vh_launch.upload(launch.data(), launch.size(), st);
        vh_part.alloc((size_t)n_chunks * 64);
        const int nvh = (int)c_off.size() - 1;
        std::vector<RowDesc> hd((size_t)std::max(nvh, 1));
        HIP_CHECK(hipMemcpyAsync(hd.data(), desc.ptr, (size_t)nvh * sizeof(RowDesc), hipMemcpyDeviceToHost, st));
        HIP_CHECK(hipStreamSynchronize(st));
        std::vector<VhWork> work(launch.size());
        for (size_t b = 0; b < launch.size(); b++) {
            VhWork &w = work[b];
            const int c = launch[b];
            w.pad_ = 0;
            if (c < 0) { w.vi = -1; w.row = 0; w.cnt = 0; w.chunk = 0; w.st = 0; continue; }
            w.vi = c_row[c]; w.row = hd[w.vi].row; w.cnt = c_cnt[c]; w.chunk = c;
            w.st = hd[w.vi].st + (unsigned long long)c_start[c];
        }
        vh_work.upload(work.data(), work.size(), st);
        HIP_CHECK(hipStreamSynchronize(st));
    }

    void build_bins(const unsigned *lens_sorted, hipStream_t st)
    {
        for (int b = 0; b < NBINS; b++) { bin_rows[b] = 0; bin_nnz[b] = 0; }
        n_empty = 0; n_long = 0; n_gt16 = 0; n_gt96 = 0; n_gt512 = 0; n_slices = 0; h_row_sl_off.assign(1, 0);
        n_gt_low[0] = n_gt_low[1] = n_gt_low[2] = n_gt_low[3] = 0;
        std::vector<int> c_row, c_first, c_cnt, c_off(1, 0);
        std::vector<int> s_row, s_first, s_count, s_off(1, 0);
        vh_min = BIN_MIN_NNZ[BIN_VHEAVY];
        if (vh_min_env() > 0) vh_min = vh_min_env();
        else if (sizeof(real_t) == 8) {
            double nnz513 = 0;
            for (int q = 0; q < nrows && lens_sorted[q] >= 513u; q++) nnz513 += (double)lens_sorted[q];
            const bool gram = (switches().vh != 0) ? switches().vh == 2 : gram_pays(nnz513, n_other, opp_row_bytes_hint);
            if (gram && opp_row_bytes_hint <= 16 * 4 * sizeof(real_t)) vh_min = 513;
        }
        long long vh_total = 0;
        for (int q = 0; q < nrows && (long long)lens_sorted[q] >= vh_min; q++) vh_total += (long long)lens_sorted[q];
        slice_len = (vh_total < (long long)GRAM_SLICE * 1024) ? 256 : GRAM_SLICE;
        for (int q = 0; q < nrows; q++) {
            const long long l = (long long)lens_sorted[q];
            if (l > LONG_ROW) n_long++;
            if (l > 16) n_gt16++;
            if (l > 96) n_gt96++;
            if (l > 512) n_gt512++;
            for (int w = 0; w < 4; w++) if (l > (long long)CG_NT_LOW * 8 * (1 << w)) n_gt_low[w]++;
            const int b = bin_of(l);
            if (b < 0) { n_empty++; continue; }
            if (b == BIN_VHEAVY) {
                const int CHN = TILE * VH_CHUNK_TILES;
                for (long long f = 0; f < l; f += CHN) {
                    c_row.push_back(bin_rows[b]); c_first.push_back((int)f); c_cnt.push_back((int)std::min<long long>(CHN, l - f));
                }
                c_off.push_back((int)c_row.size());
                const int nsl = (int)((l + slice_len - 1) / slice_len);
                const int per = (int)((((l + nsl - 1) / nsl) + 15) / 16 * 16);
                for (long long f = 0; f < l; f += per) {
                    s_row.push_back(bin_rows[b]); s_first.push_back((int)f); s_count.push_back((int)std::min<long long>(per, l - f));
                }
                s_off.push_back((int)s_row.size());
            }
            bin_rows[b]++; bin_nnz[b] += (size_t)l;
        }
        int acc = 0;
        for (int b = 0; b < NBINS; b++) { bin_first[b] = acc; acc += bin_rows[b]; }
        n_nonempty = acc;
        max_nnz = nrows ? (int)lens_sorted[0] : 0;
        if (bin_rows[BIN_VHEAVY]) {
            const int nvh = bin_rows[BIN_VHEAVY];
            set_vh_chunks(c_row, c_first, c_cnt, c_off, std::vector<int>(), st);
            vh_done.alloc(nvh); vh_r_old.alloc(nvh);
            vh_r.alloc((size_t)nvh * 64); vh_p.alloc((size_t)nvh * 64);
            n_slices = (int)s_row.size();
            sl_vrow.upload(s_row.data(), s_row.size(), st);
            sl_first.upload(s_first.data(), s_first.size(), st);
            sl_count.upload(s_count.data(), s_count.size(), st);
            row_sl_off.upload(s_off.data(), s_off.size(), st);
            h_row_sl_off = s_off;
            gram_part.alloc((size_t)n_slices * GRAM_PART);
        }
        HIP_CHECK(hipStreamSynchronize(st));
    }
};

struct DeviceInfo {
    int device = 0;
    int num_cus = 256;
    hipStream_t stream = nullptr;
    DevBuf<real_t> cg_gfull, cg_rconst;
    DevBuf<real_t> tile_init;
    DevBuf<int> row_counter;
    DevBuf<real_t> potrs_inv, potrs_tmp;
    DevBuf<real_t> potrs_ref;
    DevBuf<real_t> gemm_ws;
    hipStream_t aux_stream = nullptr;
    hipEvent_t fork_ev = nullptr, join_ev = nullptr;
    hipStream_t eig_stream_ = nullptr;
    hipEvent_t eig_fork = nullptr;
    hipStream_t eig_stream()
    {
        if (!eig_stream_) HIP_CHECK(hipStreamCreateWithFlags(&eig_stream_, hipStreamNonBlocking));
        return eig_stream_;
    }
    mutable bool nonneg_now = false;
    mutable int max_cd_steps = 100;
    mutable real_t l1_now = 0;
    mutable real_t l1_last_now = 0;
    mutable real_t l1_scale = 1;
    DeviceInfo() = default;
    DeviceInfo(const DeviceInfo &) = delete;
    DeviceInfo &operator=(const DeviceInfo &) = delete;
    ~DeviceInfo()
    {
        if (eig_fork) (void)hipEventDestroy(eig_fork);
        if (eig_stream_) (void)hipStreamDestroy(eig_stream_);
        if (fork_ev) (void)hipEventDestroy(fork_ev);
        if (join_ev) (void)hipEventDestroy(join_ev);
        for (int i = 0; i < MAX_BIN_STREAMS; i++) {
            if (bin_join[i]) (void)hipEventDestroy(bin_join[i]);
            if (i > 0 && bin_streams[i]) (void)hipStreamDestroy(bin_streams[i]);
        }
        if (aux_stream) (void)hipStreamDestroy(aux_stream);
        if (stream) (void)hipStreamDestroy(stream);
    }
    void ensure_aux()
    {
        if (aux_stream) return;
        HIP_CHECK(hipStreamCreateWithFlags(&aux_stream, hipStreamNonBlocking));
        HIP_CHECK(hipEventCreateWithFlags(&fork_ev, hipEventDisableTiming));
        HIP_CHECK(hipEventCreateWithFlags(&join_ev, hipEventDisableTiming));
    }
    static constexpr int MAX_BIN_STREAMS = 5;
    hipStream_t bin_streams[MAX_BIN_STREAMS] = {nullptr, nullptr, nullptr, nullptr, nullptr};
    hipEvent_t bin_join[MAX_BIN_STREAMS] = {nullptr, nullptr, nullptr, nullptr, nullptr};
    void ensure_bin_streams(int n)
    {
        ensure_aux();
        bin_streams[0] = aux_stream;
        if (!bin_join[0]) HIP_CHECK(hipEventCreateWithFlags(&bin_join[0], hipEventDisableTiming));
        for (int i = 1; i < n && i < MAX_BIN_STREAMS; i++) {
            if (!bin_streams[i]) HIP_CHECK(hipStreamCreateWithFlags(&bin_streams[i], hipStreamNonBlocking));
            if (!bin_join[i]) HIP_CHECK(hipEventCreateWithFlags(&bin_join[i], hipEventDisableTiming));
        }
    }
};

struct EventPair { hipEvent_t a, b; };
struct BinTimers {
    std::vector<EventPair> ev[NBINS];
    void clear()
    {
        for (auto &v : ev) {
            for (auto &p : v) { (void)hipEventDestroy(p.a); (void)hipEventDestroy(p.b); }
            v.clear();
        }
    }
};

template <bool TRANSA>
inline void launch_gemm(const DeviceInfo &dev, int M, int N, int K, real_t alpha, const real_t *A, size_t lda,
                        const real_t *B, size_t ldb, real_t *C, size_t ldc)
{
    if (M <= 0 || N <= 0) return;
    {
        DeviceInfo &d = const_cast<DeviceInfo &>(dev);
        const int bm = (M + GEMM_BM - 1) / GEMM_BM, bn = (N + GEMM_BN - 1) / GEMM_BN;
        int nsplit = 1;
        if ((long long)bm * bn < 2LL * dev.num_cus && K >= 4096)
            nsplit = (int)std::min<long long>((K + 255) / 256, std::max<long long>(1, (4LL * dev.num_cus) / ((long long)bm * bn)));
        int kchunk = (std::max(K, 1) + nsplit - 1) / nsplit;
        kchunk = (kchunk + GEMM_BK - 1) / GEMM_BK * GEMM_BK;
        nsplit = (std::max(K, 1) + kchunk - 1) / kchunk;
        const dim3 grid(bn, bm, nsplit);
        if (nsplit == 1) {
            hipLaunchKernelGGL((gemm_mfma_kernel<real_t, TRANSA>), grid, dim3(256), 0, dev.stream, M, N, K, kchunk, alpha, A, lda, B, ldb, C, ldc,
                               (size_t)0);
        } else {
            const size_t ss = (size_t)M * N;
            d.gemm_ws.alloc_at_least(ss * nsplit);
            hipLaunchKernelGGL((gemm_mfma_kernel<real_t, TRANSA>), grid, dim3(256), 0, dev.stream, M, N, K, kchunk, alpha, A, lda, B, ldb,
                               d.gemm_ws.ptr, (size_t)N, ss);
            hipLaunchKernelGGL(gemm_splitk_reduce_kernel<real_t>, dim3((unsigned)((ss + 255) / 256)), dim3(256), 0, dev.stream, d.gemm_ws.ptr, ss,
                               nsplit, M, N, C, ldc);
        }
        HIP_CHECK(hipGetLastError());
        return;
    }
}

struct GramWorkspace {
    DevBuf<real_t> partial;
};

inline void launch_gram(const DeviceInfo &dev, GramWorkspace &ws, const real_t *B, size_t ldb, int n, int k,
                        real_t *out, real_t scale, real_t add_diag)
{
    if (k <= 64) {
        int nblocks = std::max(1, std::min(dev.num_cus * 2, (n + 127) / 128));
        int rpb = (n + nblocks - 1) / nblocks;
        nblocks = (n + rpb - 1) / rpb;
        if (nblocks < 1) nblocks = 1;
        size_t need = (size_t)nblocks * k * k;
        if (ws.partial.n < need) ws.partial.alloc(need);
        const int rem = (sizeof(real_t) == 8 && k > 48 && k <= 52) ? k - 48 : 0;
        switch (rem) {
#define CMF_GRAM_REM(R) case R: hipLaunchKernelGGL((gram_mfma_partial_kernel<real_t, R>), dim3(nblocks), dim3(256), 0, dev.stream, B, ldb, n, k, rpb, ws.partial.ptr); break;
            CMF_GRAM_REM(1) CMF_GRAM_REM(2) CMF_GRAM_REM(3) CMF_GRAM_REM(4)
#undef CMF_GRAM_REM
            default: hipLaunchKernelGGL((gram_mfma_partial_kernel<real_t, 0>), dim3(nblocks), dim3(256), 0, dev.stream, B, ldb, n, k, rpb, ws.partial.ptr); break;
        }
        hipLaunchKernelGGL(gram_reduce_kernel<real_t>, dim3((k * k + GRAM_RED_ENT - 1) / GRAM_RED_ENT), dim3(256), 0, dev.stream,
                           ws.partial.ptr, nblocks, k * k, out, scale, add_diag, k);
    } else {
        launch_gemm<true>(dev, k, k, n, scale, B, ldb, B, ldb, out, (size_t)k);
        if (add_diag != 0)
            hipLaunchKernelGGL(add_diag_kernel<real_t>, dim3((k + 255) / 256), dim3(256), 0, dev.stream, out, k, 0, k, add_diag);
    }
    HIP_CHECK(hipGetLastError());
}

struct CgCall {
    real_t *A; size_t lda;
    const real_t *B; size_t ldb;
    int k;
    const real_t *bias_sub;
    const real_t *BtB;
    real_t lam, lam_last;
    bool scale_lam, scale_bias_const;
    int max_cg_steps;
    bool implicit;
    bool precond = false;
    int koff = 0, kc = 0;
    const real_t *CtC = nullptr, *UC = nullptr;
    real_t w_side = 0;
    int rows_with_u = 0, p_side = 0;
    bool scale_lam_sideinfo = false;
    const SparseShard *X2 = nullptr;
    const real_t *C2 = nullptr;
    const real_t *Bi = nullptr, *BiTBi = nullptr;
    int ki = 0;
    real_t w_imp = 0;
    const real_t *gsum = nullptr;
    int skip_first = 0;
    const real_t *Gx = nullptr, *rconst_x = nullptr;
    size_t ldr_x = 0;
    const real_t *values_override = nullptr, *weights_override = nullptr;
    bool gx_all_rows = false;
    const real_t *wsum_override = nullptr;
};

enum class CgVariant { Auto, Generic };
CgVariant cg_variant_from_env();

constexpr int NCOUNTER_SETS = 2 * NBINS + 2;
constexpr size_t ROW_COUNTER_INTS = 64 + (size_t)NCOUNTER_SETS * CG_NCOUNTERS * CG_COUNTER_STRIDE;
inline size_t cg_counter_offset(int bin) { return 64 + (size_t)bin * CG_NCOUNTERS * CG_COUNTER_STRIDE; }

__global__ void __launch_bounds__(256) poison_lds_kernel(int words)
{
    extern __shared__ unsigned int poison_words[];
    volatile unsigned int *w = poison_words;
    for (int e = threadIdx.x; e < words; e += 256) w[e] = 0xFFFFFFFFu;
}
inline void poison_lds(hipStream_t st, int num_cus)
{
    if (!switches().poison_lds) return;
    constexpr int BYTES = 80 * 1024;
    static thread_local bool attr_set = false;
    if (!attr_set) {
        HIP_CHECK(hipFuncSetAttribute((const void *)poison_lds_kernel, hipFuncAttributeMaxDynamicSharedMemorySize, BYTES));
        attr_set = true;
    }
    hipLaunchKernelGGL(poison_lds_kernel, dim3(num_cus * 4), dim3(256), BYTES, st, BYTES / 4);
    HIP_CHECK(hipGetLastError());
}

template <int S, bool IMPLICIT, int W, int RPB, bool GRAMX = false, int NRES_ = 0, int NTSEL = 0>
inline void launch_cg_bin(const DeviceInfo &dev, CgParams<real_t> P, int first, int count, BinTimers *tm, int bin, hipStream_t st, int counter_set = -1)
{
    if (count <= 0) return;
    EventPair ev{nullptr, nullptr};
    if (tm) {
        HIP_CHECK(hipEventCreate(&ev.a));
        HIP_CHECK(hipEventCreate(&ev.b));
        HIP_CHECK(hipEventRecord(ev.a, st));
    }
    poison_lds(st, dev.num_cus);
    P.order += first;
    P.desc += first;
    P.nrows = count;
    P.counter = dev.row_counter.ptr + cg_counter_offset(counter_set >= 0 ? counter_set : bin);
    constexpr int threads = 64 * W * RPB;
    size_t smem = (((IMPLICIT || GRAMX) ? (size_t)gram_elems<real_t>(S) : 0) + (size_t)RPB * 2 * W * 64) * sizeof(real_t);
    auto kern = cg_rows_kernel<real_t, S, IMPLICIT, W, RPB, GRAMX, NRES_, NTSEL>;
    static thread_local int bpc_dev[MAX_DEVICES] = {0};
    int &blocks_per_cu = bpc_dev[std::min(std::max(dev.device, 0), MAX_DEVICES - 1)];
    if (blocks_per_cu == 0) {
        if (smem > 48 * 1024)
            HIP_CHECK(hipFuncSetAttribute((const void *)kern, hipFuncAttributeMaxDynamicSharedMemorySize, (int)smem));
        int nb = 0;
        HIP_CHECK(hipOccupancyMaxActiveBlocksPerMultiprocessor(&nb, kern, threads, smem));
        blocks_per_cu = std::max(1, nb);
    }
    int teams_needed = (count + RPB - 1) / RPB;
    int grid = std::min(teams_needed, dev.num_cus * blocks_per_cu);
    hipLaunchKernelGGL(kern, dim3(grid), dim3(threads), smem, st, P);
    HIP_CHECK(hipGetLastError());
    if (tm) {
        HIP_CHECK(hipEventRecord(ev.b, st));
        tm->ev[bin].push_back(ev);
    }
}

template <int S, bool IMPLICIT, bool GRAMX = false>
inline void launch_cg_tiny(const DeviceInfo &dev, CgParams<real_t> P, int first, int count, BinTimers *tm, hipStream_t st, int n_gt16)
{
    if (count <= 0) return;
    EventPair ev{nullptr, nullptr};
    if (tm) {
        HIP_CHECK(hipEventCreate(&ev.a));
        HIP_CHECK(hipEventCreate(&ev.b));
        HIP_CHECK(hipEventRecord(ev.a, st));
    }
    poison_lds(st, dev.num_cus);
    constexpr bool tiny16_on = true;
    const int count_le16 = std::min(count, std::max(0, first + count - std::max(first, n_gt16)));
    size_t smem = ((IMPLICIT || GRAMX) ? (size_t)gram_elems<real_t>(S) : 0) * sizeof(real_t);
    const int di = std::min(std::max(dev.device, 0), MAX_DEVICES - 1);
    CgParams<real_t> P1 = P;
    P1.order += first;
    P1.desc += first;
    P1.nrows = count;
    P1.counter = dev.row_counter.ptr + cg_counter_offset(BIN_TINY);
    {
        const bool mixed = tiny16_on && count_le16 > 0;
        auto kern = mixed ? cg_rows_tiny_kernel<real_t, S, IMPLICIT, GRAMX, 0> : cg_rows_tiny_kernel<real_t, S, IMPLICIT, GRAMX, 4>;
        static thread_local int bpc_dev[MAX_DEVICES][2] = {{0}};
        int &blocks_per_cu = bpc_dev[di][mixed ? 1 : 0];
        if (blocks_per_cu == 0) {
            int nb = 0;
            HIP_CHECK(hipOccupancyMaxActiveBlocksPerMultiprocessor(&nb, kern, 256, smem));
            blocks_per_cu = std::max(1, nb);
        }
        const int grid = std::min((count + 3) / 4, dev.num_cus * blocks_per_cu);
        hipLaunchKernelGGL(kern, dim3(grid), dim3(256), smem, st, P1);
    }
    HIP_CHECK(hipGetLastError());
    if (tm) {
        HIP_CHECK(hipEventRecord(ev.b, st));
        tm->ev[BIN_TINY].push_back(ev);
    }
}

void launch_gram_wave(dim3 grid, hipStream_t st, const CgParams<real_t> &P, const GramParams<real_t> &G, bool implicit, int rem);

template <bool GRAMX>
inline bool vh_takes_gram(int k, const SparseShard &X)
{
    if (GRAMX || k > 16 * GRAM_NTT) return false;
    return (switches().vh != 0) ? switches().vh == 2 : X.prefer_gram((size_t)k * sizeof(real_t));
}

template <int S, bool IMPLICIT, bool GRAMX = false>
inline void launch_cg_vheavy(const DeviceInfo &dev_, CgParams<real_t> P, const SparseShard &X, BinTimers *tm, hipStream_t st)
{
    const int nvh = X.bin_rows[BIN_VHEAVY];
    if (nvh <= 0) return;
    struct { hipStream_t stream; int num_cus; } dev{st, dev_.num_cus};
    EventPair ev{nullptr, nullptr};
    if (tm) {
        HIP_CHECK(hipEventCreate(&ev.a));
        HIP_CHECK(hipEventCreate(&ev.b));
        HIP_CHECK(hipEventRecord(ev.a, dev.stream));
    }
    if (vh_takes_gram<GRAMX>(P.k, X)) {
        GramParams<real_t> G;
        G.sl_vrow = X.sl_vrow.ptr; G.sl_first = X.sl_first.ptr; G.sl_count = X.sl_count.ptr; G.row_sl_off = X.row_sl_off.ptr;
        G.part = X.gram_part.ptr; G.n_slices = X.n_slices; G.nvh = nvh;
        P.nrows = nvh;
#ifdef CMF_CG_DEBUG
        if (switches().debug_ticks) {
            static unsigned long long *d_t = nullptr;
            unsigned long long h[4];
            if (d_t == nullptr) { HIP_CHECK(hipMalloc((void **)&d_t, sizeof(h))); HIP_CHECK(hipMemset(d_t, 0, sizeof(h))); }
            else {
                HIP_CHECK(hipDeviceSynchronize());
                HIP_CHECK(hipMemcpy(h, d_t, sizeof(h), hipMemcpyDeviceToHost));
                if (h[1] > 0)
                    fprintf(stderr, "gram_wave: %.0f ticks per wave, %llu waves, %llu slices, %llu nnz: %.1f ticks per nnz and wave\n",
                            (double)h[0] / h[1], h[1], h[2], h[3], (double)h[0] / (double)h[3]);
                HIP_CHECK(hipMemset(d_t, 0, sizeof(h)));
            }
            G.ticks = d_t;
        }
#endif
        poison_lds(dev.stream, dev.num_cus);
        const bool slice_kernel = switches().gram_slice;
        if (slice_kernel)
            hipLaunchKernelGGL((gram_slice_kernel<real_t, IMPLICIT>), dim3(std::min(X.n_slices, dev.num_cus * 2)), dim3(64 * GRAM_NW), 0,
                           dev.stream, P, G);
        else {
            const dim3 gw(std::min((X.n_slices + 3) / 4, dev.num_cus * 4));
            const int rem = (sizeof(real_t) == 8) ? P.k - 16 * (GRAM_NTT - 1) : 0;
            launch_gram_wave(gw, dev.stream, P, G, IMPLICIT, rem);
        }
        poison_lds(dev.stream, dev.num_cus);
        hipLaunchKernelGGL((gram_cg_kernel<real_t, IMPLICIT>), dim3(std::min(nvh, dev.num_cus * 8)), dim3(256), 0, dev.stream, P, G);
        HIP_CHECK(hipGetLastError());
        if (tm) {
            HIP_CHECK(hipEventRecord(ev.b, dev.stream));
            tm->ev[BIN_VHEAVY].push_back(ev);
        }
        return;
    }
    VhState<real_t> V;
    V.r = X.vh_r.ptr; V.p = X.vh_p.ptr; V.r_old = X.vh_r_old.ptr; V.done = X.vh_done.ptr; V.part = X.vh_part.ptr;
    V.chunk_row = X.vh_chunk_row.ptr; V.chunk_start = X.vh_chunk_start.ptr; V.chunk_cnt = X.vh_chunk_cnt.ptr;
    V.chunk_off = X.vh_chunk_off.ptr; V.launch = X.vh_launch.ptr; V.work = X.vh_work.ptr;
    V.nvh = nvh; V.nchunks = X.n_chunks; V.nlaunch = X.n_launch;
    P.nrows = nvh;
    poison_lds(dev.stream, dev.num_cus);
    const dim3 gp(X.n_launch), bp(64 * VH_CHUNK_TILES), gu(nvh), bu(64 * VH_UPD_WAVES);
    hipLaunchKernelGGL((vh_pass_kernel<real_t, S, IMPLICIT, 0>), gp, bp, 0, dev.stream, P, V);
    hipLaunchKernelGGL((vh_update_kernel<real_t, IMPLICIT, 0, GRAMX>), gu, bu, 0, dev.stream, P, V);
    for (int step = 0; step < P.max_cg_steps; step++) {
        hipLaunchKernelGGL((vh_pass_kernel<real_t, S, IMPLICIT, 1>), gp, bp, 0, dev.stream, P, V);
        hipLaunchKernelGGL((vh_update_kernel<real_t, IMPLICIT, 1, GRAMX>), gu, bu, 0, dev.stream, P, V);
    }
    HIP_CHECK(hipGetLastError());
    if (tm) {
        HIP_CHECK(hipEventRecord(ev.b, dev.stream));
        tm->ev[BIN_VHEAVY].push_back(ev);
    }
}

inline int cg_bin_streams()
{
    const int n = switches().bins_par;
    return std::min(std::max(n, 1), DeviceInfo::MAX_BIN_STREAMS + 1);
}

template <int S, bool IMPLICIT, int W, int RPB, bool GRAMX>
inline void launch_cg_bin_by_tile(const DeviceInfo &dev, const CgParams<real_t> &P, const SparseShard &X, int first, int count, BinTimers *tm, int bin,
                                  hipStream_t st)
{
#ifdef CMFREC_HIP_FLOAT
    constexpr bool by_tile = S >= CMF_CG_NT_MIN_S && CMF_CG_NT_F32 && W <= 4;
#else
    constexpr bool by_tile = S >= CMF_CG_NT_MIN_S && S <= CG_NTSEL_MAX_S && (W == 1 || W == 4 || W == 8);
#endif
    if (count <= 0) return;
    if constexpr (by_tile) {
        if (switches().nt_split) {
            const int n_hi = std::min(count, std::max(0, X.n_gt_low[W == 1 ? 0 : W == 2 ? 1 : W == 4 ? 2 : 3] - first));
            EventPair ev{nullptr, nullptr};
            if (tm) { HIP_CHECK(hipEventCreate(&ev.a)); HIP_CHECK(hipEventCreate(&ev.b)); HIP_CHECK(hipEventRecord(ev.a, st)); }
            launch_cg_bin<S, IMPLICIT, W, RPB, GRAMX, 0, 2>(dev, P, first, n_hi, nullptr, bin, st);
            launch_cg_bin<S, IMPLICIT, W, RPB, GRAMX, 0, 1>(dev, P, first + n_hi, count - n_hi, nullptr, bin, st, NBINS + 2 + bin);
            if (tm) { HIP_CHECK(hipEventRecord(ev.b, st)); tm->ev[bin].push_back(ev); }
            return;
        }
    }
    launch_cg_bin<S, IMPLICIT, W, RPB, GRAMX>(dev, P, first, count, tm, bin, st);
}

template <int S, bool IMPLICIT, bool GRAMX>
inline void launch_cg_any_bin(const DeviceInfo &dev, const CgParams<real_t> &P, const SparseShard &X, BinTimers *tm, int bin, hipStream_t st)
{
    const int first = X.bin_first[bin], count = X.bin_rows[bin];
    switch (bin) {
        case BIN_HEAVY:
#ifdef CMFREC_HIP_FLOAT
            {
                const int n_long8 = std::min(count, std::max(0, X.n_gt512 - first));
                EventPair ev{nullptr, nullptr};
                if (tm) { HIP_CHECK(hipEventCreate(&ev.a)); HIP_CHECK(hipEventCreate(&ev.b)); HIP_CHECK(hipEventRecord(ev.a, st)); }
                launch_cg_bin<S, IMPLICIT, 8, 1, GRAMX>(dev, P, first, n_long8, nullptr, bin, st);
                launch_cg_bin<S, IMPLICIT, 4, 1, GRAMX, 2>(dev, P, first + n_long8, count - n_long8, nullptr, bin, st, NBINS);
                if (tm) { HIP_CHECK(hipEventRecord(ev.b, st)); tm->ev[bin].push_back(ev); }
                break;
            }
#endif
            launch_cg_bin_by_tile<S, IMPLICIT, 8, 1, GRAMX>(dev, P, X, first, count, tm, bin, st); break;
        case BIN_MED4: launch_cg_bin_by_tile<S, IMPLICIT, 4, 1, GRAMX>(dev, P, X, first, count, tm, bin, st); break;
        case BIN_MED2: launch_cg_bin_by_tile<S, IMPLICIT, 2, 1, GRAMX>(dev, P, X, first, count, tm, bin, st); break;
        default: launch_cg_bin_by_tile<S, IMPLICIT, 1, 4, GRAMX>(dev, P, X, first, count, tm, bin, st); break;
    }
}

template <int S, bool IMPLICIT, bool GRAMX = false>
inline void launch_cg_S(const DeviceInfo &dev, const CgParams<real_t> &P, const SparseShard &X, BinTimers *tm)
{
    if (dev.row_counter.n < ROW_COUNTER_INTS) const_cast<DeviceInfo &>(dev).row_counter.alloc(ROW_COUNTER_INTS);
    HIP_CHECK(hipMemsetAsync(dev.row_counter.ptr, 0, ROW_COUNTER_INTS * sizeof(int), dev.stream));
    const bool vh_aside = X.bin_rows[BIN_VHEAVY] > 0 && X.vh_runs_aside(dev.num_cus) && !vh_takes_gram<GRAMX>(P.k, X);
    const bool alt = X.is_part;
    DeviceInfo &d = const_cast<DeviceInfo &>(dev);
    const int npar = cg_bin_streams();
    if (npar > 1 && !(vh_aside || alt)) {
        d.ensure_bin_streams(npar - 1);
        hipStream_t ss[DeviceInfo::MAX_BIN_STREAMS + 1];
        ss[0] = dev.stream;
        for (int i = 1; i < npar; i++) ss[i] = d.bin_streams[i - 1];
        HIP_CHECK(hipEventRecord(d.fork_ev, dev.stream));
        for (int i = 1; i < npar; i++) HIP_CHECK(hipStreamWaitEvent(ss[i], d.fork_ev, 0));
        static const double row_equiv[NBINS] = {0.0, 126.0, 7.0, 7.0, 0.0, 11.5};
        double cost[NBINS], load[DeviceInfo::MAX_BIN_STREAMS + 1] = {0, 0, 0, 0, 0, 0};
        int order_b[NBINS];
        for (int b = 0; b < NBINS; b++) {
            cost[b] = (double)X.bin_nnz[b] + row_equiv[b] * (double)X.bin_rows[b];
            order_b[b] = b;
        }
        std::sort(order_b, order_b + NBINS, [&](int a, int b2) { return cost[a] > cost[b2]; });
        for (int q = 0; q < NBINS; q++) {
            const int b = order_b[q];
            if (X.bin_rows[b] <= 0) continue;
            int si = 0;
            for (int i = 1; i < npar; i++) if (load[i] < load[si]) si = i;
            load[si] += cost[b];
            if (b == BIN_VHEAVY) launch_cg_vheavy<S, IMPLICIT, GRAMX>(dev, P, X, tm, ss[si]);
            else if (b == BIN_TINY) launch_cg_tiny<S, IMPLICIT, GRAMX>(dev, P, X.bin_first[BIN_TINY], X.bin_rows[BIN_TINY], tm, ss[si], X.n_gt16);
            else launch_cg_any_bin<S, IMPLICIT, GRAMX>(dev, P, X, tm, b, ss[si]);
        }
        for (int i = 1; i < npar; i++) {
            HIP_CHECK(hipEventRecord(d.bin_join[i - 1], ss[i]));
            HIP_CHECK(hipStreamWaitEvent(dev.stream, d.bin_join[i - 1], 0));
        }
        return;
    }
    if (vh_aside || alt) {
        d.ensure_aux();
        HIP_CHECK(hipEventRecord(d.fork_ev, dev.stream));
        HIP_CHECK(hipStreamWaitEvent(d.aux_stream, d.fork_ev, 0));
    }
    hipStream_t s0 = dev.stream, s1 = alt ? d.aux_stream : dev.stream;
    launch_cg_vheavy<S, IMPLICIT, GRAMX>(dev, P, X, tm, (vh_aside || (alt && X.is_part)) ? d.aux_stream : dev.stream);
    launch_cg_any_bin<S, IMPLICIT, GRAMX>(dev, P, X, tm, BIN_HEAVY, s0);
    launch_cg_any_bin<S, IMPLICIT, GRAMX>(dev, P, X, tm, BIN_MED4, s1);
    launch_cg_any_bin<S, IMPLICIT, GRAMX>(dev, P, X, tm, BIN_MED2, s0);
    launch_cg_any_bin<S, IMPLICIT, GRAMX>(dev, P, X, tm, BIN_LIGHT, s1);
    launch_cg_tiny<S, IMPLICIT, GRAMX>(dev, P, X.bin_first[BIN_TINY], X.bin_rows[BIN_TINY], tm, s0, X.n_gt16);
    if (vh_aside || alt) {
        HIP_CHECK(hipEventRecord(d.join_ev, d.aux_stream));
        HIP_CHECK(hipStreamWaitEvent(dev.stream, d.join_ev, 0));
    }
}

template <int NF, bool IMPLICIT>
inline void launch_cg_generic(const DeviceInfo &dev, CgParams<real_t> P, const SparseShard &X, int first = 0, bool all_rows = false)
{
    int count = (P.kc > 0 || P.Bi != nullptr || all_rows) ? X.nrows : X.n_nonempty;
    if (count <= first) return;
    const int nteam = std::min(count, X.bin_first[BIN_MED2]);
    const int nvh = std::min(nteam, X.bin_rows[BIN_VHEAVY]);
    poison_lds(dev.stream, dev.num_cus);
    if (nvh > first) {
        P.row_first = first; P.nrows = nvh;
        hipLaunchKernelGGL((cg_rows_generic_kernel<real_t, NF, IMPLICIT, 16>), dim3(std::min(nvh - first, dev.num_cus * 2)), dim3(1024), 0,
                           dev.stream, P);
    }
    if (nteam > std::max(nvh, first)) {
        P.row_first = std::max(nvh, first); P.nrows = nteam;
        hipLaunchKernelGGL((cg_rows_generic_kernel<real_t, NF, IMPLICIT, 4>), dim3(std::min(nteam - P.row_first, dev.num_cus * 8)), dim3(256), 0,
                           dev.stream, P);
    }
    if (count > std::max(nteam, first)) {
        P.row_first = std::max(nteam, first); P.nrows = count;
        int grid = std::min((count - P.row_first + 3) / 4, dev.num_cus * 8);
        hipLaunchKernelGGL((cg_rows_generic_kernel<real_t, NF, IMPLICIT, 1>), dim3(grid), dim3(256), 0, dev.stream, P);
    }
    HIP_CHECK(hipGetLastError());
}

#ifdef CMF_CG_TICKS
inline unsigned long long *cg_ticks_buffer()
{
    static unsigned long long *buf = nullptr;
    if (buf == nullptr) {
        HIP_CHECK(hipMalloc((void **)&buf, 32 * sizeof(unsigned long long)));
        HIP_CHECK(hipMemset(buf, 0, 32 * sizeof(unsigned long long)));
    }
    return buf;
}
#endif

inline int launch_cg(const DeviceInfo &dev, const CgCall &c, const SparseShard &X, BinTimers *tm = nullptr)
{
    CgParams<real_t> P;
    P.A = c.A; P.lda = c.lda; P.B = c.B; P.ldb = c.ldb; P.k = c.k;
    P.indptr = X.p.ptr; P.indices = X.i.ptr; P.values = X.v.ptr;
    P.bias_sub = c.bias_sub; P.order = X.order.ptr; P.desc = X.desc.ptr; P.nrows = 0; P.BtB = c.BtB;
    if (!c.implicit && X.weighted()) { P.weights = X.w.ptr; P.wsum = X.wsum.ptr; }
    P.lam = c.lam; P.lam_last = c.lam_last;
    P.scale_lam = c.scale_lam; P.scale_bias_const = c.scale_bias_const;
    P.max_cg_steps = c.max_cg_steps;
    P.precond = c.precond ? 1 : 0;
    P.koff = c.koff; P.kc = c.kc; P.CtC = c.CtC; P.UC = c.UC; P.w_side = c.w_side;
    P.rows_with_u = c.rows_with_u; P.p_side = c.p_side; P.scale_lam_sideinfo = c.scale_lam_sideinfo ? 1 : 0;
    if (c.X2) { P.indptr2 = c.X2->p.ptr; P.indices2 = c.X2->i.ptr; P.values2 = c.X2->v.ptr; P.C2 = c.C2; }
    P.Bi = c.Bi; P.BiTBi = c.BiTBi; P.ki = c.ki; P.w_imp = c.w_imp;
#ifdef CMF_CG_DEBUG
    P.dbg = switches().debug_skip;
#endif
#ifdef CMF_CG_TICKS
    P.ticks = cg_ticks_buffer();
#endif
    const int S = (c.k + 7) / 8;
    if (c.values_override != nullptr) P.values = c.values_override;
    if (c.weights_override != nullptr) { P.weights = c.weights_override; P.wsum = X.wsum_naz.ptr; }
    if (c.wsum_override != nullptr) P.wsum = c.wsum_override;
    if (c.Gx != nullptr && (c.kc > 0 || c.X2 != nullptr || c.Bi != nullptr)) {
        if (c.implicit || c.skip_first != 0) {
            g_last_error = "cmfrec_hip: block CG with a shared matrix: the explicit model";
            return 2;
        }
        P.BtB = c.Gx; P.rconst = c.rconst_x; P.ldr = c.ldr_x; P.gx = c.gx_all_rows ? 2 : 1;
        const int NFb = (c.koff + c.k + 63) / 64;
        switch (NFb) {
            case 1: launch_cg_generic<1, false>(dev, P, X, 0, true); return 0;
            case 2: launch_cg_generic<2, false>(dev, P, X, 0, true); return 0;
            case 3: launch_cg_generic<3, false>(dev, P, X, 0, true); return 0;
            default: break;
        }
        g_last_error = "cmfrec_hip: block CG with a shared matrix: at most 192 unknowns per row";
        return 2;
    }
    if (c.Gx != nullptr && c.precond) {
        if (c.implicit || c.kc > 0 || c.Bi != nullptr || c.koff != 0 || c.skip_first != 0 || c.X2 != nullptr) {
            g_last_error = "cmfrec_hip: preconditioned CG with a shared matrix: plain explicit rows";
            return 2;
        }
        P.BtB = c.Gx; P.rconst = c.rconst_x; P.ldr = c.ldr_x; P.gx = 1;
        const int NFx = (c.k + 63) / 64;
        switch (NFx) {
            case 1: launch_cg_generic<1, false>(dev, P, X, 0, c.gx_all_rows); return 0;
            case 2: launch_cg_generic<2, false>(dev, P, X, 0, c.gx_all_rows); return 0;
            case 3: launch_cg_generic<3, false>(dev, P, X, 0, c.gx_all_rows); return 0;
            default: break;
        }
        g_last_error = "cmfrec_hip: preconditioned CG with a shared matrix: at most 192 unknowns per row";
        return 2;
    }
    if (c.Gx != nullptr) {
        if (c.implicit || c.precond || S > 8 || c.kc > 0 || c.Bi != nullptr || c.koff != 0 || c.skip_first != 0) {
            g_last_error = "cmfrec_hip: CG with a shared matrix: plain explicit rows of at most 64 unknowns, no preconditioner";
            return 2;
        }
        P.BtB = c.Gx; P.rconst = c.rconst_x; P.ldr = c.ldr_x;
#define CMF_XCASE(SS) case SS: launch_cg_S<SS, false, true>(dev, P, X, tm); break;
        switch (S) {
            CMF_XCASE(1) CMF_XCASE(2) CMF_XCASE(3) CMF_XCASE(4)
            CMF_XCASE(5) CMF_XCASE(6) CMF_XCASE(7) CMF_XCASE(8)
        }
#undef CMF_XCASE
        HIP_CHECK(hipGetLastError());
        return 0;
    }
    const bool block = (c.kc > 0 || c.Bi != nullptr);
    const bool tiled_block = block && cg_variant_from_env() != CgVariant::Generic && !c.implicit && c.koff == 0 && !c.precond && c.skip_first == 0 &&
                             S <= 8 && c.X2 == nullptr && (c.kc == 0 || (c.rows_with_u >= X.nrows && c.CtC != nullptr && c.UC != nullptr)) &&
                             (c.Bi == nullptr || (c.gsum != nullptr && c.BiTBi != nullptr)) && c.kc <= c.k && c.ki <= c.k;
    if (tiled_block) {
        DeviceInfo &d = const_cast<DeviceInfo &>(dev);
        d.cg_gfull.alloc_at_least((size_t)c.k * c.k);
        d.cg_rconst.alloc_at_least((size_t)std::max(X.nrows, 1) * c.k);
        hipLaunchKernelGGL(block_gram_kernel<real_t>, dim3((c.k * c.k + 255) / 256), dim3(256), 0, dev.stream, c.CtC, c.kc, c.w_side, c.BiTBi,
                           c.ki, c.w_imp, c.k, d.cg_gfull.ptr);
        hipLaunchKernelGGL(block_rconst_kernel<real_t>, dim3((unsigned)(((size_t)X.nrows * c.k + 255) / 256)), dim3(256), 0, dev.stream, c.UC, c.kc,
                           c.w_side, c.gsum, c.ki, c.w_imp, c.k, (size_t)X.nrows, d.cg_rconst.ptr);
        P.BtB = d.cg_gfull.ptr; P.rconst = d.cg_rconst.ptr; P.ldr = (size_t)c.k;
#define CMF_BCASE(SS) case SS: launch_cg_S<SS, false, true>(dev, P, X, tm); break;
        switch (S) {
            CMF_BCASE(1) CMF_BCASE(2) CMF_BCASE(3) CMF_BCASE(4)
            CMF_BCASE(5) CMF_BCASE(6) CMF_BCASE(7) CMF_BCASE(8)
        }
#undef CMF_BCASE
        if (X.nrows > X.n_nonempty) {
            CgParams<real_t> Pe = P;
            Pe.BtB = c.BtB; Pe.rconst = nullptr;
            Pe.row_first = X.n_nonempty; Pe.nrows = X.nrows;
            const int cnt = X.nrows - X.n_nonempty;
            const int NFe = (c.koff + c.k + 63) / 64;
            const int grid = std::min((cnt + 3) / 4, dev.num_cus * 8);
            switch (NFe) {
                case 1: hipLaunchKernelGGL((cg_rows_generic_kernel<real_t, 1, false, 1>), dim3(grid), dim3(256), 0, dev.stream, Pe); break;
                default: hipLaunchKernelGGL((cg_rows_generic_kernel<real_t, 2, false, 1>), dim3(grid), dim3(256), 0, dev.stream, Pe); break;
            }
        }
        HIP_CHECK(hipGetLastError());
        return 0;
    }
    const bool generic = cg_variant_from_env() == CgVariant::Generic || S > 8 || c.precond || c.kc > 0 || c.Bi != nullptr || c.skip_first > 0;
    if (!generic) {
#define CMF_CASE(SS)                                                        \
    case SS:                                                                \
        if (c.implicit) launch_cg_S<SS, true>(dev, P, X, tm);               \
        else            launch_cg_S<SS, false>(dev, P, X, tm);              \
        return 0;
        switch (S) {
            CMF_CASE(1) CMF_CASE(2) CMF_CASE(3) CMF_CASE(4)
            CMF_CASE(5) CMF_CASE(6) CMF_CASE(7) CMF_CASE(8)
        }
#undef CMF_CASE
    }
    const int NF = (c.koff + c.k + 63) / 64;
#define CMF_GCASE(NN)                                                       \
    case NN:                                                                \
        if (c.implicit) launch_cg_generic<NN, true>(dev, P, X, c.skip_first);  \
        else            launch_cg_generic<NN, false>(dev, P, X, c.skip_first); \
        return 0;
    switch (NF) {
        CMF_GCASE(1) CMF_GCASE(2) CMF_GCASE(3) CMF_GCASE(4) CMF_GCASE(5)
    }
#undef CMF_GCASE
    g_last_error = "cmfrec_hip: CG path supports k <= 320 per solved matrix";
    return 2;
}

}
```

cmfrec_amd/csrc/device_base.hpp:

```cpp
#pragma once
#include <hip/hip_runtime.h>
#include <cstdio>
#include <cstdlib>
#include <cstring>
#include <functional>
#include <new>
#include <string>

#include "../../include/cmfrec_hip.h"

namespace cmfhip {

extern thread_local std::string g_last_error;
extern thread_local int g_last_rc;

struct HipError {
    int code;
};

inline void hip_check(hipError_t e, const char *what, const char *file, int line)
{
    if (e == hipSuccess) return;
    char buf[512];
    snprintf(buf, sizeof buf, "cmfrec_hip: %s failed: %s (%s:%d)", what, hipGetErrorString(e), file, line);
    g_last_error = buf;
    fprintf(stderr, "%s\n", buf);
    throw HipError{e == hipErrorOutOfMemory ? 1 : 4};
}
#define HIP_CHECK(x) ::cmfhip::hip_check((x), #x, __FILE__, __LINE__)

inline int guarded(const std::function<int()> &f)
{
    try {
        return f();
    } catch (const HipError &e) {
        return e.code;
    } catch (const std::bad_alloc &) {
        g_last_error = "cmfrec_hip: host out of memory";
        return 1;
    }
}

struct Switches {
    bool poison_lds = false;
    int vh_min = 0;
    int vh = 0;
    bool gram_slice = false;
    int bins_par = 2;
    bool nt_split = true;
    bool cg_generic = false;
    int chol = 0;
    int parts_coop = 1;
    int chol_wg = 2;
    int gramk = -1;
    int gramk_batch = 0;
    int lowrank = -1;
    bool topn_wide = false;
    int topn_tiles = 0;
    bool eig_jacobi = false;
    int debug_skip = 0;
    bool debug_ticks = false;
    int newrows_block_rows = 0;
    void reload()
    {
        auto str = [](const char *n) -> const char * { const char *v = getenv(n); return (v != nullptr && v[0] != 0) ? v : nullptr; };
        auto num = [&](const char *n, int dflt) -> int { const char *v = str(n); return v ? atoi(v) : dflt; };
        poison_lds = str("CMFREC_HIP_POISON_LDS") != nullptr;
        vh_min = num("CMFREC_HIP_VH_MIN", 0);
        const char *v = str("CMFREC_HIP_VH");
        vh = !v ? 0 : strcmp(v, "stream") == 0 ? 1 : strcmp(v, "gram") == 0 ? 2 : 1;
        v = str("CMFREC_HIP_GRAM_KERNEL"); gram_slice = v && strcmp(v, "slice") == 0;
        bins_par = num("CMFREC_HIP_BINS_PAR", 2);
        nt_split = num("CMFREC_HIP_NT_SPLIT", 1) != 0;
        v = str("CMFREC_HIP_CG_KERNEL"); cg_generic = v && strcmp(v, "generic") == 0;
        v = str("CMFREC_HIP_CHOL"); chol = !v ? 0 : strcmp(v, "rows") == 0 ? 1 : strcmp(v, "noslices") == 0 ? 2 : 0;
        parts_coop = num("CMFREC_HIP_PARTS_COOP", 1);
        chol_wg = num("CMFREC_HIP_CHOL_WG", 2);
        if (chol_wg == 1) chol_wg = 2;
        gramk = num("CMFREC_HIP_GRAMK", -1);
        gramk_batch = num("CMFREC_HIP_GRAMK_BATCH", 0);
        lowrank = num("CMFREC_HIP_LOWRANK", -1);
        v = str("CMFREC_HIP_TOPN"); topn_wide = v && strcmp(v, "wide") == 0;
        topn_tiles = num("CMFREC_HIP_TOPN_TILES", 0);
        v = str("CMFREC_HIP_EIG"); eig_jacobi = v && strcmp(v, "jacobi") == 0;
        debug_skip = num("CMFREC_HIP_CG_SKIP", num("CMFREC_HIP_CHOL_SKIP", num("CMFREC_HIP_WAVE_SKIP", 0)));
        debug_ticks = str("CMFREC_HIP_GRAM_TICKS") != nullptr || str("CMFREC_HIP_CHOL_TICKS") != nullptr;
        newrows_block_rows = num("CMFREC_HIP_NEWROWS_BLOCK_ROWS", 0);
    }
};
inline Switches &switches_mut() { static Switches sw; static bool first = (sw.reload(), true); (void)first; return sw; }
inline const Switches &switches() { return switches_mut(); }

template <typename T>
struct DevBuf {
    T *ptr = nullptr;
    size_t n = 0;
    bool owned = true;
    DevBuf() = default;
    DevBuf(const DevBuf &) = delete;
    DevBuf &operator=(const DevBuf &) = delete;
    ~DevBuf() { release(); }
    void release()
    {
        if (ptr && owned) (void)hipFree(ptr);
        ptr = nullptr;
        n = 0;
    }
    void alloc(size_t count)
    {
        release();
        n = count;
        owned = true;
        if (count) HIP_CHECK(hipMalloc((void **)&ptr, count * sizeof(T)));
        if (count && switches().poison_lds) {
            HIP_CHECK(hipMemset(ptr, 0xFF, count * sizeof(T)));
            HIP_CHECK(hipDeviceSynchronize());
        }
    }
    void alloc_at_least(size_t count)
    {
        if (n < count) alloc(count);
    }
    void upload(const T *host, size_t count, hipStream_t st)
    {
        if (count > n) alloc(count);
        if (count) HIP_CHECK(hipMemcpyAsync(ptr, host, count * sizeof(T), hipMemcpyDefault, st));
    }
    void download(T *host, size_t count, hipStream_t st) const
    {
        if (count) HIP_CHECK(hipMemcpyAsync(host, ptr, count * sizeof(T), hipMemcpyDeviceToHost, st));
    }
};

void open_device(int device, int *device_id, int *num_cus, hipStream_t *stream);

}
```

cmfrec_amd/csrc/gram_cg_kernels.hpp:

```cpp
#pragma once
#include <hip/hip_runtime.h>
#include <stdint.h>

#include "cg_kernels.hpp"
#include "chol_kernels.hpp"
#include "lanes.hpp"

namespace cmfhip {

constexpr int GRAM_NTT = 4;
constexpr int GRAM_NTILES = GRAM_NTT * (GRAM_NTT + 1) / 2;
constexpr int GRAM_PART = GRAM_NTILES * 256 + 64;
constexpr int GRAM_CH = 32;
constexpr int GRAM_NW = 4;

template <typename T>
struct GramParams {
    const int *sl_vrow;
    const int *sl_first;
    const int *sl_count;
    const int *row_sl_off;
    T *part;
    int n_slices, nvh;
#ifdef CMF_CG_DEBUG
    unsigned long long *ticks = nullptr;
#endif
};

template <typename T>
__device__ __forceinline__ T treduce8_rows(const T (&c)[8], int lane)
{
    T n4[4], n2[2];
#pragma unroll
    for (int i = 0; i < 4; i++) n4[i] = lanes::tswap32_add(c[i], c[4 + i]);
#pragma unroll
    for (int i = 0; i < 2; i++) n2[i] = lanes::tswap16_add(n4[i], n4[2 + i]);
    T n1 = ((lane & 8) ? n2[1] : n2[0]) + lanes::recv_xor8(n2[0], n2[1]);
    n1 += lanes::xor4(n1);
    n1 += lanes::xor2(n1);
    n1 += lanes::xor1(n1);
    return n1;
}

template <typename T, bool IMPLICIT>
__global__ void __launch_bounds__(64 * GRAM_NW, 2)
gram_slice_kernel(const CgParams<T> P, const GramParams<T> Gp)
{
    using Mf = CholMfma<T>;
    using vec = typename Mf::vec;
    constexpr int NTT = GRAM_NTT, NW = GRAM_NW, CH = GRAM_CH;
    constexpr int ldc = 16 * NTT + 16;
    constexpr int NTALL = GRAM_NTILES;
    constexpr int TPW = (NTALL + NW - 1) / NW;
    constexpr int RPW = CH / NW;
    static_assert(RPW == 8, "treduce8_rows");
    __shared__ T ring[2 * CH * ldc];
    __shared__ T wsc[2 * CH];
    __shared__ T vpart[NW * 64];
    const int kt = P.k;
    const int tid = threadIdx.x, lane = tid & 63, wave = tid >> 6, lm = lane & 15;
    int offa[TPW], offb[TPW];
#pragma unroll
    for (int tt = 0; tt < TPW; tt++) {
        const int t = min(wave + NW * tt, NTALL - 1);
        offa[tt] = 16 * tile_bi(t, NTT);
        offb[tt] = 16 * tile_bj(t, NTT);
    }
    const int scol = (lane < kt) ? lane : 0;
    const bool svalid = lane < kt;
    const int myrow = lane >> 3;

    for (int sl = blockIdx.x; sl < Gp.n_slices; sl += gridDim.x) {
        const RowDesc d = P.desc[Gp.sl_vrow[sl]];
        const size_t st = d.st + (size_t)Gp.sl_first[sl];
        const int nnz = Gp.sl_count[sl];
        const T *arow = P.A + (size_t)d.row * P.lda;
        const T a_l = (IMPLICIT && svalid) ? arow[lane] : T(0);
        vec acc[TPW];
#pragma unroll
        for (int tt = 0; tt < TPW; tt++) acc[tt] = vec{0, 0, 0, 0};
        T racc = T(0);
        T pre[RPW];
        int idn[RPW];
        int idx_l = 0; T x_l = T(0), xw_l = T(0), g_l = T(1);
        T gw_l = T(1);
        int nr_rows = 0, nr_idx = 0;
        auto load_idx = [&](int c0) {
            nr_idx = min(CH, nnz - c0);
#pragma unroll
            for (int i = 0; i < RPW; i++) idn[i] = P.indices[st + c0 + min(RPW * wave + i, nr_idx - 1)];
            const size_t e = st + c0 + min(RPW * wave + myrow, nr_idx - 1);
            idx_l = P.indices[e]; x_l = P.values[e]; g_l = entry_weight<T, IMPLICIT>(P, e);
        };
        auto load_rows = [&]() {
            nr_rows = nr_idx;
#pragma unroll
            for (int i = 0; i < RPW; i++) pre[i] = P.B[(size_t)idn[i] * P.ldb + scol];
            xw_l = x_l;
            if (!IMPLICIT && P.bias_sub != nullptr) xw_l -= P.bias_sub[idx_l];
            gw_l = g_l;
            if (!IMPLICIT) xw_l *= g_l;
        };
        if (nnz > 0) { load_idx(0); load_rows(); }
        if (nnz > CH) load_idx(CH);
        __syncthreads();
        for (int c0 = 0, slot = 0; c0 < nnz; c0 += CH, slot ^= 1) {
            T *Bs = ring + slot * CH * ldc;
            T bv[RPW], prod[RPW];
#pragma unroll
            for (int i = 0; i < RPW; i++) {
                bv[i] = (RPW * wave + i < nr_rows && svalid) ? pre[i] : T(0);
                Bs[(RPW * wave + i) * ldc + lane] = bv[i];
                if (lane < ldc - 64) Bs[(RPW * wave + i) * ldc + 64 + lane] = T(0);
                prod[i] = bv[i] * a_l;
            }
            const bool live_l = (RPW * wave + myrow < nr_rows);
            T wv = live_l ? xw_l : T(0);
            if (IMPLICIT) wv -= treduce8_rows(prod, lane);
            if ((lane & 7) == 0) wsc[slot * CH + RPW * wave + myrow] = live_l ? (IMPLICIT ? xw_l : gw_l) : T(0);
#pragma unroll
            for (int i = 0; i < RPW; i++) racc += bcast_lane(wv, 8 * i) * bv[i];
            __syncthreads();
            if (c0 + CH < nnz) load_rows();
            if (c0 + 2 * CH < nnz) load_idx(c0 + 2 * CH);
#pragma unroll
            for (int q = 0; q < CH / 4; q++) {
                const int rr = 4 * q + (lane >> 4);
                const T *brow = Bs + rr * ldc + lm;
                const T w = wsc[slot * CH + rr];
                T opa[TPW], opb[TPW];
#pragma unroll
                for (int tt = 0; tt < TPW; tt++) { opa[tt] = brow[offa[tt]]; opb[tt] = brow[offb[tt]]; }
#pragma unroll
                for (int tt = 0; tt < TPW; tt++) acc[tt] = Mf::mma(opa[tt] * w, opb[tt], acc[tt]);
                __builtin_amdgcn_sched_barrier(0);
            }
        }
        T *out = Gp.part + (size_t)sl * GRAM_PART;
#pragma unroll
        for (int tt = 0; tt < TPW; tt++) {
            const int t = wave + NW * tt;
            if (t < NTALL) {
#pragma unroll
                for (int r = 0; r < 4; r++) out[t * 256 + r * 64 + lane] = acc[tt][r];
            }
        }
        __syncthreads();
        vpart[wave * 64 + lane] = racc;
        __syncthreads();
        if (tid < 64) {
            T vs = T(0);
#pragma unroll
            for (int w2 = 0; w2 < NW; w2++) vs += vpart[w2 * 64 + tid];
            out[NTALL * 256 + tid] = (tid < kt) ? vs : T(0);
        }
    }
}

#ifndef GW_SLABS_F32
#define GW_SLABS_F32 4
#endif
#ifndef GW_SLABS_F64
#define GW_SLABS_F64 4
#endif
template <typename T> constexpr int gw_slabs() { return sizeof(T) == 4 ? GW_SLABS_F32 : GW_SLABS_F64; }

constexpr int GW_REM = 4;
template <typename T, bool IMPLICIT, int REM = 0, bool FULLK = false>
__global__ void __launch_bounds__(256, 2)
gram_wave_kernel(const CgParams<T> P, const GramParams<T> Gp)
{
    using Mf = CholMfma<T>;
    using vec = typename Mf::vec;
    constexpr int NTT = GRAM_NTT, NTALL = GRAM_NTILES, NS = gw_slabs<T>(), GRP = 4 * NS;
    constexpr bool REMV = REM > 0;
    constexpr int NTF = REMV ? NTT - 1 : NTT;
    static_assert(REM >= 0 && REM <= GW_REM, "remainder columns");
    const int kt = P.k;
    const int lane = threadIdx.x & 63, wave = threadIdx.x >> 6;
    const int kc = lane >> 4, lm = lane & 15;
    size_t coff[NTT];
    bool cok[NTT];
#pragma unroll
    for (int cb = 0; cb < NTT; cb++) { cok[cb] = (16 * cb + lm) < kt; coff[cb] = (size_t)min(16 * cb + lm, kt - 1); }
    const unsigned ldb_bytes = (unsigned)(P.ldb * sizeof(T));
#ifdef CMF_CG_DEBUG
    const unsigned long long tick0 = __builtin_readcyclecounter();
    unsigned long long nsl_ = 0, nnz_ = 0;
#endif

    for (int sl = blockIdx.x * 4 + wave; sl < Gp.n_slices; sl += gridDim.x * 4) {
        const RowDesc d = P.desc[Gp.sl_vrow[sl]];
        const size_t st = d.st + (size_t)Gp.sl_first[sl];
        const int nnz = Gp.sl_count[sl];
#ifdef CMF_CG_DEBUG
        nsl_++; nnz_ += nnz;
#endif
        T a_c[NTT];
#pragma unroll
        for (int cb = 0; cb < NTT; cb++) a_c[cb] = (IMPLICIT && cok[cb]) ? P.A[(size_t)d.row * P.lda + coff[cb]] : T(0);
        vec acc[NTALL];
#pragma unroll
        for (int t = 0; t < NTALL; t++) acc[t] = vec{0, 0, 0, 0};
        T racc[NTT];
#pragma unroll
        for (int cb = 0; cb < NTT; cb++) racc[cb] = T(0);
        T cacc[REMV ? REM : 1][NTT];
#pragma unroll
        for (int c = 0; c < (REMV ? REM : 1); c++)
#pragma unroll
            for (int cb = 0; cb < NTT; cb++) cacc[c][cb] = T(0);

        auto load_entries = [&](int c0, int &idx, T &x, T &okf) {
            const int e = c0 + (lane & (GRP - 1));
            const bool ok = e < nnz;
            const size_t pos = st + (size_t)max(min(e, nnz - 1), 0);
            idx = P.indices[pos];
            x = P.values[pos];
            if (!IMPLICIT && P.bias_sub != nullptr) x -= P.bias_sub[idx];
            okf = ok ? entry_weight<T, IMPLICIT>(P, pos) : T(0);
        };
        auto load_slabs = [&](int idx, T (&slab)[NS][NTT]) {
#pragma unroll
            for (int q = 0; q < NS; q++) {
                const unsigned it = (unsigned)__shfl(idx, 4 * q + kc);
                const T *rp = reinterpret_cast<const T *>(reinterpret_cast<const char *>(P.B) + (unsigned long long)it * ldb_bytes);
                if constexpr (FULLK) {
                    const T *rl = rp + lm;
#pragma unroll
                    for (int cb = 0; cb < NTT; cb++) slab[q][cb] = rl[16 * cb];
                } else if constexpr (REMV) {
                    const T *rl = rp + lm;
#pragma unroll
                    for (int cb = 0; cb < NTF; cb++) slab[q][cb] = rl[16 * cb];
                    slab[q][NTT - 1] = rp[coff[NTT - 1]];
                } else {
#pragma unroll
                    for (int cb = 0; cb < NTT; cb++) slab[q][cb] = rp[coff[cb]];
                }
            }
        };
        int idx_c, idx_n;
        T x_c, ok_c, x_n, ok_n;
        T bufA[NS][NTT], bufB[NS][NTT];
        load_entries(0, idx_c, x_c, ok_c);
        load_slabs(idx_c, bufA);
        load_entries(GRP, idx_n, x_n, ok_n);
        auto group = [&](int c0, T (&S_)[NS][NTT], T (&N_)[NS][NTT]) {
            load_slabs(idx_n, N_);
            int idx_nn; T x_nn, ok_nn;
            load_entries(c0 + 2 * GRP, idx_nn, x_nn, ok_nn);
#pragma unroll
            for (int q = 0; q < NS; q++) {
                const T x = __shfl(x_c, 4 * q + kc), okf = __shfl(ok_c, 4 * q + kc);
                T wG, wv;
                if (IMPLICIT) {
                    T dp = T(0);
#pragma unroll
                    for (int cb = 0; cb < NTT; cb++) dp += S_[q][cb] * a_c[cb];
                    dp += lanes::xor1(dp); dp += lanes::xor2(dp); dp += lanes::qxor4(dp); dp += lanes::xor8(dp);
                    wG = x * okf;
                    wv = (x - dp) * okf;
                } else {
                    wG = okf;
                    wv = x * okf;
                }
                T sa[NTT];
#pragma unroll
                for (int cb = 0; cb < NTT; cb++) {
                    racc[cb] += wv * S_[q][cb];
                    sa[cb] = wG * S_[q][cb];
                }
                static_for<0, NTALL>([&](auto tc) {
                    constexpr int t = decltype(tc)::value, bi = tile_bi(t, NTT), bj = tile_bj(t, NTT);
                    if constexpr (bj < NTF) acc[t] = Mf::mma(sa[bi], S_[q][bj], acc[t]);
                });
                if constexpr (REMV) {
                    static_for<0, REM>([&](auto cc) {
                        constexpr int c = decltype(cc)::value;
                        const T we = wG * lanes::row_bcast16<c>(S_[q][NTT - 1]);
#pragma unroll
                        for (int cb = 0; cb < NTT; cb++) cacc[c][cb] += we * S_[q][cb];
                    });
                }
            }
            idx_c = idx_n; x_c = x_n; ok_c = ok_n;
            idx_n = idx_nn; x_n = x_nn; ok_n = ok_nn;
        };
        for (int c0 = 0; c0 < nnz; c0 += 2 * GRP) {
            group(c0, bufA, bufB);
            if (c0 + GRP < nnz) group(c0 + GRP, bufB, bufA);
        }
        T *out = Gp.part + (size_t)sl * GRAM_PART;
        static_for<0, NTALL>([&](auto tc) {
            constexpr int t = decltype(tc)::value;
            if constexpr (tile_bj(t, NTT) < NTF) {
#pragma unroll
                for (int r = 0; r < 4; r++) out[t * 256 + r * 64 + lane] = acc[t][r];
            }
        });
        if constexpr (REMV) {
            static_for<0, REM>([&](auto cc) {
                constexpr int c = decltype(cc)::value;
                static_for<0, NTT>([&](auto cbc) {
                    constexpr int cb = decltype(cbc)::value;
                    constexpr int t = cb * NTT - cb * (cb - 1) / 2 + (NTT - 1 - cb);
                    T v = lanes::tswap32_add(cacc[c][cb], cacc[c][cb]);
                    v = lanes::tswap16_add(v, v);
                    if (kc == 0) out[t * 256 + Mf::cidx(lm, c)] = v;
                });
            });
        }
#pragma unroll
        for (int cb = 0; cb < NTT; cb++) {
            T v = lanes::tswap32_add(racc[cb], racc[cb]);
            v = lanes::tswap16_add(v, v);
            if (kc == 0) out[NTALL * 256 + 16 * cb + lm] = cok[cb] ? v : T(0);
        }
    }
#ifdef CMF_CG_DEBUG
    if (Gp.ticks != nullptr && lane == 0) {
        atomicAdd(&Gp.ticks[0], __builtin_readcyclecounter() - tick0);
        atomicAdd(&Gp.ticks[1], 1ull); atomicAdd(&Gp.ticks[2], nsl_); atomicAdd(&Gp.ticks[3], nnz_);
    }
#endif
}

template <typename T, bool IMPLICIT>
__global__ void __launch_bounds__(256)
gram_cg_kernel(const CgParams<T> P, const GramParams<T> Gp)
{
    using Mf = CholMfma<T>;
    constexpr int NTT = GRAM_NTT, NTALL = GRAM_NTILES, LDM = 65;
    __shared__ T M[64 * LDM];
    __shared__ T vec_s[64];
    const int kt = P.k;
    const int tid = threadIdx.x, lane = tid & 63;
    for (int vr = blockIdx.x; vr < Gp.nvh; vr += gridDim.x) {
        const RowDesc d = P.desc[vr];
        T *arow = P.A + (size_t)d.row * P.lda;
        const int s0 = Gp.row_sl_off[vr], s1 = Gp.row_sl_off[vr + 1];
        T lam = P.lam, lam_last = P.lam_last;
        if (!IMPLICIT && P.scale_lam) {
            const T mult = row_lam_mult(P, d.row, d.nnz);
            lam *= mult;
            if (!P.scale_bias_const) lam_last *= mult;
        }
        __syncthreads();
        if (kt < 64)
            for (int e = tid; e < 64 * LDM; e += 256) M[e] = T(0);
        if (kt < 64) __syncthreads();
        constexpr int EPT = NTALL * 256 / 256, SB = 4;
        T sacc[EPT];
#pragma unroll
        for (int q = 0; q < EPT; q++) sacc[q] = T(0);
        for (int sl = s0; sl < s1; sl += SB) {
            T t8[EPT][SB];
#pragma unroll
            for (int q = 0; q < EPT; q++)
#pragma unroll
                for (int u = 0; u < SB; u++) t8[q][u] = (sl + u < s1) ? Gp.part[(size_t)(sl + u) * GRAM_PART + tid + 256 * q] : T(0);
#pragma unroll
            for (int q = 0; q < EPT; q++)
#pragma unroll
                for (int u = 0; u < SB; u++) sacc[q] += t8[q][u];
        }
#pragma unroll
        for (int q = 0; q < EPT; q++) {
            const int e = tid + 256 * q;
            T s = sacc[q];
            const int t = e >> 8, r = (e >> 6) & 3, l = e & 63;
            const int i = 16 * tile_bi(t, NTT) + Mf::row_of(l, r), j = 16 * tile_bj(t, NTT) + (l & 15);
            if (j >= i && j < kt) {
                if (IMPLICIT) s += P.BtB[(size_t)i * kt + j];
                if (i == j) s += (!IMPLICIT && i == kt - 1) ? lam_last : lam;
                M[i * LDM + j] = s;
                M[j * LDM + i] = s;
            }
        }
        T v = T(0);
        if (tid < 64) {
            for (int sl = s0; sl < s1; sl += 8) {
                T t8[8];
#pragma unroll
                for (int u = 0; u < 8; u++) t8[u] = (sl + u < s1) ? Gp.part[(size_t)(sl + u) * GRAM_PART + NTALL * 256 + tid] : T(0);
#pragma unroll
                for (int u = 0; u < 8; u++) v += t8[u];
            }
        }
        __syncthreads();
        if (tid < 64) {
            const bool live = lane < kt;
            T a = live ? arow[lane] : T(0);
            auto mul = [&](T x) {
                vec_s[lane] = x;
                asm volatile("s_waitcnt lgkmcnt(0)" ::: "memory");
                T y0 = T(0), y1 = T(0), y2 = T(0), y3 = T(0);
                const T *mrow = M + lane * LDM;
#pragma unroll
                for (int c = 0; c < 64; c += 4) {
                    y0 += mrow[c] * vec_s[c]; y1 += mrow[c + 1] * vec_s[c + 1];
                    y2 += mrow[c + 2] * vec_s[c + 2]; y3 += mrow[c + 3] * vec_s[c + 3];
                }
                asm volatile("s_waitcnt lgkmcnt(0)" ::: "memory");
                return (y0 + y1) + (y2 + y3);
            };
            const T Ma = mul(a);
            T r = live ? v - Ma : T(0);
            T p = r;
            T r_old = lanes::wave_sum(r * r);
            if (r_old > (T)1e-12) {
                for (int step = 0; step < P.max_cg_steps; step++) {
                    const T Mp = mul(p);
                    const T Ap = live ? Mp : T(0);
                    const T alpha = cg_div(r_old, lanes::wave_sum(Ap * p));
                    a += alpha * p; r -= alpha * Ap;
                    const T r_new = lanes::wave_sum(r * r);
                    if (r_new <= (T)1e-8) break;
                    p = p * cg_div(r_new, r_old) + r;
                    r_old = r_new;
                }
            }
            if (live) arow[lane] = a;
        }
    }
}

}
```

Before: 165.1 million.

## Overlap next-row tile gather with final CG pass and skip last residual update

Adds an optional early-gather path (CMF_CG_EARLY_GATHER, default 0) that issues the next row's B-tile loads interleaved with the FMA accumulation of the current row's final CG pass, so that gather latency is hidden behind compute. Independently of that flag, the CG loops now skip the residual and search-direction update on the last step, which always runs in the gram CG kernel and also in the main CG kernel. It also adds an env-controlled team cap (CMFREC_HIP_CG_TEAMS) that remaps row descriptors on the host. The early-gather path holds extra tile registers, which can reduce occupancy.

After: 167.4 million (median of 6 runs). 1.01x the previous value.

```diff
diff --git a/cmfrec_amd/csrc/cg_kernels.hpp b/cmfrec_amd/csrc/cg_kernels.hpp
--- a/cmfrec_amd/csrc/cg_kernels.hpp
+++ b/cmfrec_amd/csrc/cg_kernels.hpp
@@ -272,6 +272,26 @@
     }
 };
 
+#ifndef CMF_CG_EARLY_GATHER
+#define CMF_CG_EARLY_GATHER 0
+#endif
+struct NoAfter {
+    template <typename TAG> __device__ __forceinline__ void operator()(TAG) const {}
+};
+template <int S, typename ACC>
+__device__ __forceinline__ void pin_acc(ACC &out)
+{
+#pragma unroll
+    for (int s = 0; s < S; s++) asm volatile("" : "+v"(out.v[s]));
+}
+template <int TS, typename T, int S, typename TILE>
+__device__ __forceinline__ void load_tile_slot(TILE &tile, const char *base, unsigned ldb_bytes, unsigned it, int col_last)
+{
+    const T *rp = reinterpret_cast<const T *>(base + (unsigned long long)it * ldb_bytes);
+#pragma unroll
+    for (int s = 0; s < S; s++) tile.set(TS, s, rp[(s < S - 1) ? 8 * s : col_last]);
+}
+
 template <typename T, int S, int NT = 8>
 __device__ __forceinline__ void load_tile(RegTile<T, S> &tile, const T *__restrict__ Bm, size_t ldb,
                                           int k, int my_idx, int cnt, int lane)
@@ -323,9 +343,9 @@
     return (P.weights != nullptr) ? P.weights[pos] : T(1);
 }
 
-template <int S, bool IMPLICIT, int MODE, int NT = 8, bool INIT = false>
+template <int S, bool IMPLICIT, int MODE, int NT = 8, bool INIT = false, typename AFTER = NoAfter>
 __device__ __forceinline__ void tile_pass_f32(const RegTile<float, S> &tile, const float (&vrep)[S], float x, bool valid,
-                                          PassAcc<float> &out, int lane, float g = 1.f)
+                                          PassAcc<float> &out, int lane, float g = 1.f, AFTER after = AFTER())
 {
     static_assert(NT % 2 == 0, "single precision: the entries of a lane group travel in pairs");
     float c[8];
@@ -342,24 +362,36 @@
     wts[0] = lanes::bcast8<0>(w); wts[1] = lanes::bcast8<1>(w); wts[2] = lanes::bcast8<2>(w); wts[3] = lanes::bcast8<3>(w);
     if (NT > 4) { wts[4] = lanes::bcast8<4>(w); wts[5] = lanes::bcast8<5>(w); }
     if (NT > 6) { wts[6] = lanes::bcast8<6>(w); wts[7] = lanes::bcast8<7>(w); }
+    if constexpr (std::is_same<AFTER, NoAfter>::value) {
 #pragma unroll
     for (int q = 0; q < NT / 2; q++) {
         const f32x2 w2 = f32x2{wts[2 * q], wts[2 * q + 1]};
 #pragma unroll
         for (int s = 0; s < S; s++) out.v[s] = (INIT && q == 0) ? w2 * tile.v[q][s] : out.v[s] + w2 * tile.v[q][s];
     }
+    } else {
+        static_for<0, NT / 2>([&](auto qc) {
+            constexpr int q = decltype(qc)::value;
+            const f32x2 w2 = f32x2{wts[2 * q], wts[2 * q + 1]};
+#pragma unroll
+            for (int s = 0; s < S; s++) out.v[s] = (INIT && q == 0) ? w2 * tile.v[q][s] : out.v[s] + w2 * tile.v[q][s];
+            pin_acc<S>(out);
+            after(std::integral_constant<int, 2 * q>{});
+            after(std::integral_constant<int, 2 * q + 1>{});
+        });
+    }
     if constexpr (INIT) {
 #pragma unroll
         for (int s = S; s < 8; s++) out.v[s] = f32x2{0.f, 0.f};
     }
 }
 
-template <typename T, int S, bool IMPLICIT, int MODE, int NT = 8, bool INIT = false>
+template <typename T, int S, bool IMPLICIT, int MODE, int NT = 8, bool INIT = false, typename AFTER = NoAfter>
 __device__ __forceinline__ void tile_pass(const RegTile<T, S> &tile, const T (&vrep)[S], T x, bool valid,
-                                          PassAcc<T> &out, int lane, T g = T(1))
+                                          PassAcc<T> &out, int lane, T g = T(1), AFTER after = AFTER())
 {
     if constexpr (std::is_same<T, float>::value) {
-        tile_pass_f32<S, IMPLICIT, MODE, NT, INIT>(tile, vrep, x, valid, out, lane, g);
+        tile_pass_f32<S, IMPLICIT, MODE, NT, INIT, AFTER>(tile, vrep, x, valid, out, lane, g, after);
     } else {
     T c[8];
 #pragma unroll
@@ -377,10 +409,20 @@
     if (NT > 5) wts[5] = lanes::bcast8<5>(w);
     if (NT > 6) wts[6] = lanes::bcast8<6>(w);
     if (NT > 7) wts[7] = lanes::bcast8<7>(w);
+    if constexpr (std::is_same<AFTER, NoAfter>::value) {
 #pragma unroll
     for (int t = 0; t < NT; t++) {
 #pragma unroll
         for (int s = 0; s < S; s++) out.v[s] = (INIT && t == 0) ? wts[t] * tile.v[t][s] : out.v[s] + wts[t] * tile.v[t][s];
+    }
+    } else {
+        static_for<0, NT>([&](auto tc) {
+            constexpr int t = decltype(tc)::value;
+#pragma unroll
+            for (int s = 0; s < S; s++) out.v[s] = (INIT && t == 0) ? wts[t] * tile.v[t][s] : out.v[s] + wts[t] * tile.v[t][s];
+            pin_acc<S>(out);
+            after(tc);
+        });
     }
     if constexpr (INIT) {
 #pragma unroll
@@ -556,6 +598,42 @@
     RowDesc dnxt = load_desc(rnxt);
     Pre pcur = load_pre(dcur);
     int pend = issue_claim();
+    constexpr bool EARLY = CMF_CG_EARLY_GATHER != 0;
+    constexpr int NT_MAX = (NTSEL == 1) ? CG_NT_LOW : 8;
+    RegTile<T, S> tile_c;
+    RegTile<T, (NRES == 2) ? S : 1> tile2_c;
+    const char *const gbase = reinterpret_cast<const char *>(P.B + (lane & 7));
+    const unsigned gldb = (unsigned)(P.ldb * sizeof(T));
+    const int gcol_last = min((lane & 7) + 8 * (S - 1), k - 1) - (lane & 7);
+    auto gather_slot = [&](auto &tl_, auto tc, int idx_, int first_idx_, int nt_, int cnt_) {
+        constexpr int t = decltype(tc)::value;
+        if constexpr (t < NT_MAX) {
+            if (t < nt_) {
+                const unsigned it_ = (unsigned)((((lane >> 3) * nt_ + t) < cnt_) ? lanes::bcast8<t>(idx_) : first_idx_);
+                load_tile_slot<t, T, S>(tl_, gbase, gldb, it_, gcol_last);
+            }
+        }
+    };
+    struct Want { int nt0, cnt0, nt1, cnt1; };
+    auto want_of = [&](const RowDesc &d) -> Want {
+        Want w_;
+        const int nt = nt_of(d.nnz), tl = 8 * nt;
+        w_.cnt0 = min(tl, d.nnz - wr * tl);
+        w_.nt0 = (w_.cnt0 > 0 && !CMF_DBG(P, 1)) ? nt : 0;
+        w_.cnt1 = (NRES == 2) ? min(tl, d.nnz - (wr + W) * tl) : 0;
+        w_.nt1 = (w_.cnt1 > 0 && !CMF_DBG(P, 1)) ? nt : 0;
+        return w_;
+    };
+    auto gather_row = [&](const RowDesc &d, const Pre &q) {
+        const Want w_ = want_of(d);
+        const int f0 = __builtin_amdgcn_readfirstlane(q.idx);
+        static_for<0, NT_MAX>([&](auto tc) { gather_slot(tile_c, tc, q.idx, f0, w_.nt0, w_.cnt0); });
+        if constexpr (NRES == 2) {
+            const int f1 = __builtin_amdgcn_readfirstlane(q.idx2);
+            static_for<0, NT_MAX>([&](auto tc) { gather_slot(tile2_c, tc, q.idx2, f1, w_.nt1, w_.cnt1); });
+        }
+    };
+    if constexpr (EARLY) gather_row(dcur, pcur);
 #ifdef CMF_CG_TICKS
     unsigned long long tk_wait = 0, tk_pass = 0, tk_rows = 0;
     const unsigned long long tk_begin = CMF_TICK();
@@ -588,7 +666,10 @@
         T *arow = P.A + (size_t)row * P.lda;
         T a_d = pcur.a;
 
-        RegTile<T, S> tile;
+        RegTile<T, S> tile_r;
+        RegTile<T, (NRES == 2) ? S : 1> tile2_r;
+        auto &tile = [&]() -> RegTile<T, S> & { if constexpr (EARLY) return tile_c; else return tile_r; }();
+        auto &tile2 = [&]() -> RegTile<T, (NRES == 2) ? S : 1> & { if constexpr (EARLY) return tile2_c; else return tile2_r; }();
         const int ent = (lane >> 3) * NT + (lane & 7);
         const bool lane_has = (NT == 8) || (lane & 7) < NT;
         const int cnt0 = min(TL, nnz - wr * TL);
@@ -596,13 +677,12 @@
         const T g_res = pcur.g;
         bool valid_res = lane_has && ent < cnt0;
         if (CMF_DBG(P, 1)) dbg_fill_tile<8, S>(tile, (T)(pcur.idx & 3) * (T)0.001);
-        else if (cnt0 > 0) load_tile<T, S, NT>(tile, P.B, P.ldb, k, pcur.idx, cnt0, lane);
-        RegTile<T, (NRES == 2) ? S : 1> tile2;
+        else if (!EARLY && cnt0 > 0) load_tile<T, S, NT>(tile, P.B, P.ldb, k, pcur.idx, cnt0, lane);
         const int cnt1 = (NRES == 2) ? min(TL, nnz - (wr + W) * TL) : 0;
         const T x2_res = pcur.x2, g2_res = pcur.g2;
         const bool valid2_res = lane_has && ent < cnt1;
         if constexpr (NRES == 2) {
-            if (cnt1 > 0 && !CMF_DBG(P, 1)) load_tile<T, S, NT>(tile2, P.B, P.ldb, k, pcur.idx2, cnt1, lane);
+            if (!EARLY && cnt1 > 0 && !CMF_DBG(P, 1)) load_tile<T, S, NT>(tile2, P.B, P.ldb, k, pcur.idx2, cnt1, lane);
         }
         dnn = load_desc(rnn);
         pnxt = load_pre(dnxt);
@@ -613,8 +693,9 @@
         tk_wait += tk1 - tk0;
 #endif
 
-        auto run_pass = [&](T vdist, auto mode_tag, bool first) -> T {
+        auto run_pass = [&](T vdist, auto mode_tag, bool first, auto fin_tag) -> T {
             constexpr int MODE = decltype(mode_tag)::value;
+            constexpr bool FIN = decltype(fin_tag)::value && EARLY;
             asm volatile("" ::: "memory");
             T vrep[S];
             T gw[8];
@@ -622,6 +703,38 @@
             else replicate<T, S>(vdist, vrep, lane);
             PassAcc<T> acc;
             acc.zero();
+            if constexpr (FIN) {
+                if (NT < 8 || NRES == 2 || resident) {
+                    const Want nx = want_of(dnxt);
+                    const int f0 = __builtin_amdgcn_readfirstlane(pnxt.idx);
+                    auto after0 = [&](auto tc) { gather_slot(tile, tc, pnxt.idx, f0, nx.nt0, nx.cnt0); };
+                    if (cnt0 > 0 && !CMF_DBG(P, 4)) {
+                        tile_pass<T, S, IMPLICIT, MODE, NT>(tile, vrep, x_res, valid_res, acc, lane, g_res, after0);
+                        static_for<NT, NT_MAX>(after0);
+                    } else static_for<0, NT_MAX>(after0);
+                    if constexpr (NRES == 2) {
+                        const int f1 = __builtin_amdgcn_readfirstlane(pnxt.idx2);
+                        auto after1 = [&](auto tc) { gather_slot(tile2, tc, pnxt.idx2, f1, nx.nt1, nx.cnt1); };
+                        if (cnt1 > 0 && !CMF_DBG(P, 4)) {
+                            tile_pass<T, S, IMPLICIT, MODE, NT>(tile2, vrep, x2_res, valid2_res, acc, lane, g2_res, after1);
+                            static_for<NT, NT_MAX>(after1);
+                        } else static_for<0, NT_MAX>(after1);
+                    }
+                } else {
+                for (int tl = wr; tl < ntiles; tl += W) {
+                    const int cnt = min(TL, nnz - tl * TL);
+                    const bool valid = lane_has && ent < cnt;
+                    const size_t pos = st + (size_t)tl * TL + ent;
+                    int my_idx = valid ? P.indices[pos] : 0;
+                    T x = valid ? P.values[pos] : T(0);
+                    const T g = valid ? entry_weight<T, IMPLICIT>(P, pos) : T(1);
+                    if (!IMPLICIT && P.bias_sub != nullptr && valid) x -= P.bias_sub[my_idx];
+                    if (!CMF_DBG(P, 1)) load_tile<T, S, NT>(tile, P.B, P.ldb, k, my_idx, cnt, lane);
+                    if (!CMF_DBG(P, 4)) tile_pass<T, S, IMPLICIT, MODE, NT>(tile, vrep, x, valid, acc, lane, g);
+                }
+                gather_row(dnxt, pnxt);
+                }
+            } else
             if constexpr (NRES == 2) {
                 if (cnt0 > 0 && !CMF_DBG(P, 4)) tile_pass<T, S, IMPLICIT, MODE, NT>(tile, vrep, x_res, valid_res, acc, lane, g_res);
                 if (cnt1 > 0 && !CMF_DBG(P, 4)) tile_pass<T, S, IMPLICIT, MODE, NT>(tile2, vrep, x2_res, valid2_res, acc, lane, g2_res);
@@ -665,7 +778,7 @@
             return tot;
         };
 
-        T r_d = run_pass(a_d, std::integral_constant<int, 0>{}, true);
+        T r_d = run_pass(a_d, std::integral_constant<int, 0>{}, true, std::false_type{});
         r_d -= lam * a_d;
         if (!IMPLICIT && lam != lam_last && lane == k - 1) r_d -= (lam_last - lam) * a_d;
         if (GRAMX && P.rconst != nullptr && lane < k) r_d += P.rconst[(size_t)row * P.ldr + lane];
@@ -673,13 +786,14 @@
         T p_d = r_d;
         T r_old = CMF_DBG(P, 8) ? T(1) : wave_sum(r_d * r_d);
         bool done = (r_old <= (T)1e-12);
-        for (int step = 0; step < P.max_cg_steps && !done; step++) {
-            T Ap_d = run_pass(p_d, std::integral_constant<int, 1>{}, false);
+        for (int step = 0; step < P.max_cg_steps - (EARLY ? 1 : 0) && !done; step++) {
+            T Ap_d = run_pass(p_d, std::integral_constant<int, 1>{}, false, std::false_type{});
             Ap_d += lam * p_d;
             if (!IMPLICIT && lam != lam_last && lane == k - 1) Ap_d += (lam_last - lam) * p_d;
             if (lane >= k) Ap_d = T(0);
             T alpha = CMF_DBG(P, 8) ? T(0.001) : cg_div(r_old, wave_sum(Ap_d * p_d));
             a_d += alpha * p_d;
+            if (!EARLY && step == P.max_cg_steps - 1) break;
             r_d -= alpha * Ap_d;
             T r_new = CMF_DBG(P, 8) ? T(0.5) : wave_sum(r_d * r_d);
             if (r_new <= (T)1e-8) done = true;
@@ -688,10 +802,18 @@
                 r_old = r_new;
             }
         }
-        if (wr == 0 && lane < k) arow[lane] = a_d;
+        if (EARLY && P.max_cg_steps > 0 && !done) {
+            T Ap_d = run_pass(p_d, std::integral_constant<int, 1>{}, false, std::true_type{});
+            Ap_d += lam * p_d;
+            if (!IMPLICIT && lam != lam_last && lane == k - 1) Ap_d += (lam_last - lam) * p_d;
+            if (lane >= k) Ap_d = T(0);
+            const T alpha = CMF_DBG(P, 8) ? T(0.001) : cg_div(r_old, wave_sum(Ap_d * p_d));
+            a_d += alpha * p_d;
+        } else if constexpr (EARLY) gather_row(dnxt, pnxt);
 #ifdef CMF_CG_TICKS
         tk_pass += CMF_TICK() - tk1; tk_rows += (wr == 0);
 #endif
+        if (wr == 0 && lane < k) arow[lane] = a_d;
     };
     for (; rix < P.nrows; it++) {
         const int nt = nt_of(dcur.nnz);
@@ -778,9 +900,9 @@
     return q + lanes::xor1(q);
 }
 
-template <int S, bool IMPLICIT, int MODE, typename TILE, bool INIT = false>
+template <int S, bool IMPLICIT, int MODE, typename TILE, bool INIT = false, typename AFTER = NoAfter>
 __device__ __forceinline__ void tile_pass4_f32(const TILE &tile, const float (&vrep)[S], float x, bool valid,
-                                           PassAcc<float> &out, int lane, float g = 1.f)
+                                           PassAcc<float> &out, int lane, float g = 1.f, AFTER after = AFTER())
 {
     float c[4];
 #pragma unroll
@@ -794,24 +916,36 @@
     const float w = pass_weight<float, IMPLICIT, MODE>(coef, x, valid, g);
     float wts[4];
     wts[0] = lanes::bcast8<0>(w); wts[1] = lanes::bcast8<2>(w); wts[2] = lanes::bcast8<4>(w); wts[3] = lanes::bcast8<6>(w);
+    if constexpr (std::is_same<AFTER, NoAfter>::value) {
 #pragma unroll
     for (int q = 0; q < 2; q++) {
         const f32x2 w2 = f32x2{wts[2 * q], wts[2 * q + 1]};
 #pragma unroll
         for (int s = 0; s < S; s++) out.v[s] = (INIT && q == 0) ? w2 * tile.v[q][s] : out.v[s] + w2 * tile.v[q][s];
     }
+    } else {
+        static_for<0, 2>([&](auto qc) {
+            constexpr int q = decltype(qc)::value;
+            const f32x2 w2 = f32x2{wts[2 * q], wts[2 * q + 1]};
+#pragma unroll
+            for (int s = 0; s < S; s++) out.v[s] = (INIT && q == 0) ? w2 * tile.v[q][s] : out.v[s] + w2 * tile.v[q][s];
+            pin_acc<S>(out);
+            after(std::integral_constant<int, 2 * q>{});
+            after(std::integral_constant<int, 2 * q + 1>{});
+        });
+    }
     if constexpr (INIT) {
 #pragma unroll
         for (int s = S; s < 8; s++) out.v[s] = f32x2{0.f, 0.f};
     }
 }
 
-template <typename T, int S, bool IMPLICIT, int MODE, typename TILE, bool INIT = false>
+template <typename T, int S, bool IMPLICIT, int MODE, typename TILE, bool INIT = false, typename AFTER = NoAfter>
 __device__ __forceinline__ void tile_pass4(const TILE &tile, const T (&vrep)[S], T x, bool valid,
-                                           PassAcc<T> &out, int lane, T g = T(1))
+                                           PassAcc<T> &out, int lane, T g = T(1), AFTER after = AFTER())
 {
     if constexpr (std::is_same<T, float>::value) {
-        tile_pass4_f32<S, IMPLICIT, MODE, TILE, INIT>(tile, vrep, x, valid, out, lane, g);
+        tile_pass4_f32<S, IMPLICIT, MODE, TILE, INIT, AFTER>(tile, vrep, x, valid, out, lane, g, after);
     } else {
     T c[4];
 #pragma unroll
@@ -825,10 +959,20 @@
     const T w = pass_weight<T, IMPLICIT, MODE>(coef, x, valid, g);
     T wts[4];
     wts[0] = lanes::bcast8<0>(w); wts[1] = lanes::bcast8<2>(w); wts[2] = lanes::bcast8<4>(w); wts[3] = lanes::bcast8<6>(w);
+    if constexpr (std::is_same<AFTER, NoAfter>::value) {
 #pragma unroll
     for (int t = 0; t < 4; t++) {
 #pragma unroll
         for (int s = 0; s < S; s++) out.v[s] = (INIT && t == 0) ? wts[t] * tile.v[t][s] : out.v[s] + wts[t] * tile.v[t][s];
+    }
+    } else {
+        static_for<0, 4>([&](auto tc) {
+            constexpr int t = decltype(tc)::value;
+#pragma unroll
+            for (int s = 0; s < S; s++) out.v[s] = (INIT && t == 0) ? wts[t] * tile.v[t][s] : out.v[s] + wts[t] * tile.v[t][s];
+            pin_acc<S>(out);
+            after(tc);
+        });
     }
     if constexpr (INIT) {
 #pragma unroll
@@ -879,9 +1023,9 @@
     return u + lanes::xor1(u);
 }
 
-template <typename T, int S, bool IMPLICIT, int MODE, typename TILE, bool INIT = false>
+template <typename T, int S, bool IMPLICIT, int MODE, typename TILE, bool INIT = false, typename AFTER = NoAfter>
 __device__ __forceinline__ void tile_pass2(const TILE &tile, const T (&vrep)[S], T x, bool valid,
-                                           PassAcc<T> &out, int lane, T g = T(1))
+                                           PassAcc<T> &out, int lane, T g = T(1), AFTER after = AFTER())
 {
     T c[2];
     if constexpr (std::is_same<T, float>::value) {
@@ -905,6 +1049,9 @@
         const f32x2 w2 = f32x2{w0, w1};
 #pragma unroll
         for (int s = 0; s < S; s++) out.v[s] = INIT ? w2 * tile.pair0(s) : out.v[s] + w2 * tile.pair0(s);
+        if constexpr (!std::is_same<AFTER, NoAfter>::value) pin_acc<S>(out);
+        after(std::integral_constant<int, 0>{});
+        after(std::integral_constant<int, 1>{});
         if constexpr (INIT) {
 #pragma unroll
             for (int s = S; s < 8; s++) out.v[s] = f32x2{0.f, 0.f};
@@ -912,8 +1059,12 @@
     } else {
 #pragma unroll
         for (int s = 0; s < S; s++) out.v[s] = INIT ? w0 * tile.get(0, s) : out.v[s] + w0 * tile.get(0, s);
+        if constexpr (!std::is_same<AFTER, NoAfter>::value) pin_acc<S>(out);
+        after(std::integral_constant<int, 0>{});
 #pragma unroll
         for (int s = 0; s < S; s++) out.v[s] += w1 * tile.get(1, s);
+        if constexpr (!std::is_same<AFTER, NoAfter>::value) pin_acc<S>(out);
+        after(std::integral_constant<int, 1>{});
         if constexpr (INIT) {
 #pragma unroll
             for (int s = S; s < 8; s++) out.v[s] = T(0);
@@ -1061,8 +1212,36 @@
         if constexpr (NE != 2) load_tile4<T, S>(t_, Bm_, ldb_, k_, idx_, cnt_, lane_);
         else load_tile2<T, S>(t_, Bm_, ldb_, k_, idx_, cnt_, lane_);
     };
-    auto solve = [&](const RowDesc &d, const Pre &pr, const Tile &tile, auto short_tag) {
+    constexpr bool EARLY = CMF_CG_EARLY_GATHER != 0 && CMF_TINY_WAVES_PER_SIMD >= 3;
+    constexpr int NE_MAX = (NE == 2) ? 2 : 4;
+    const char *const gbase = reinterpret_cast<const char *>(P.B + (lane & 7));
+    const unsigned gldb = (unsigned)(P.ldb * sizeof(T));
+    const int gcol_last = min((lane & 7) + 8 * (S - 1), k - 1) - (lane & 7);
+    auto gather_slot = [&](Tile &tl_, auto tc, int idx_, int first_idx_, int ne_, int cnt_) {
+        constexpr int t = decltype(tc)::value;
+        if constexpr (t < NE_MAX) {
+            if (t < ne_) {
+                int its;
+                if constexpr (NE == 2) its = lanes::bcast8<(4 * t) & 7>(idx_);
+                else if constexpr (!MIX || t != 1) its = lanes::bcast8<(t == 0) ? 0 : (t == 2) ? 4 : (t == 3) ? 6 : 2>(idx_);
+                else its = (ne_ == 2) ? lanes::bcast8<4>(idx_) : lanes::bcast8<2>(idx_);
+                const unsigned it_ = (unsigned)((((lane >> 3) * ne_ + t) < cnt_) ? its : first_idx_);
+                load_tile_slot<t, T, S>(tl_, gbase, gldb, it_, gcol_last);
+            }
+        }
+    };
+    auto slots_of = [&](const RowDesc &d) -> int {
+        if (d.nnz <= 0 || CMF_DBG(P, 1)) return 0;
+        return (NE == 2 || short_row(d.nnz)) ? 2 : 4;
+    };
+    auto gather_row = [&](Tile &tl_, const RowDesc &d, const Pre &q) {
+        const int ne_ = slots_of(d);
+        const int f0 = __builtin_amdgcn_readfirstlane(q.idx);
+        static_for<0, NE_MAX>([&](auto tc) { gather_slot(tl_, tc, q.idx, f0, ne_, d.nnz); });
+    };
+    auto solve = [&](const RowDesc &d, const Pre &pr, Tile &tile, auto short_tag, auto next_tag, const RowDesc &dn, const Pre &pn) {
         constexpr bool T2 = NE == 2 || decltype(short_tag)::value;
+        constexpr bool NEXT = decltype(next_tag)::value && EARLY;
         const int nnz = d.nnz;
         T lam = P.lam, lam_last = P.lam_last;
         if (GRAMX && P.kc > 0) {
@@ -1078,17 +1257,30 @@
         }
         const bool valid = (T2 ? (lane >> 2) : (lane >> 1)) < nnz;
         T a_d = pr.a;
-        auto run_pass = [&](T vdist, auto mode_tag) -> T {
+        auto run_pass = [&](T vdist, auto mode_tag, auto fin_tag) -> T {
             constexpr int MODE = decltype(mode_tag)::value;
+            constexpr bool FIN = decltype(fin_tag)::value && NEXT;
             asm volatile("" ::: "memory");
             T vrep[S];
             T gw[8];
             if constexpr (PV) pass_vector_lds<T, S, GR>(vdist, vrep, gw, lane, &s_pv[tid >> 6][0]);
             else replicate<T, S>(vdist, vrep, lane);
             PassAcc<T> acc;
+            if constexpr (FIN) {
+                const int ne_ = slots_of(dn);
+                const int f0 = __builtin_amdgcn_readfirstlane(pn.idx);
+                auto after = [&](auto tc) { gather_slot(tile, tc, pn.idx, f0, ne_, dn.nnz); };
+                if (!CMF_DBG(P, 4)) {
+                    if constexpr (!T2) tile_pass4<T, S, IMPLICIT, MODE, Tile, true>(tile, vrep, pr.x, valid, acc, lane, pr.g, after);
+                    else {
+                        tile_pass2<T, S, IMPLICIT, MODE, Tile, true>(tile, vrep, pr.x, valid, acc, lane, pr.g, after);
+                        static_for<2, NE_MAX>(after);
+                    }
+                } else { acc.zero(); static_for<0, NE_MAX>(after); }
+            } else
             if (!CMF_DBG(P, 4)) {
-                if constexpr (!T2) tile_pass4<T, S, IMPLICIT, MODE, decltype(tile), true>(tile, vrep, pr.x, valid, acc, lane, pr.g);
-                else tile_pass2<T, S, IMPLICIT, MODE, decltype(tile), true>(tile, vrep, pr.x, valid, acc, lane, pr.g);
+                if constexpr (!T2) tile_pass4<T, S, IMPLICIT, MODE, Tile, true>(tile, vrep, pr.x, valid, acc, lane, pr.g);
+                else tile_pass2<T, S, IMPLICIT, MODE, Tile, true>(tile, vrep, pr.x, valid, acc, lane, pr.g);
             } else acc.zero();
             if constexpr (GREG) {
                 if (!CMF_DBG(P, 2)) {
@@ -1101,7 +1293,7 @@
             acc.close(out);
             return treduce8_high<T>(out, lane);
         };
-        T r_d = run_pass(a_d, std::integral_constant<int, 0>{});
+        T r_d = run_pass(a_d, std::integral_constant<int, 0>{}, std::false_type{});
         r_d -= lam * a_d;
         if (!IMPLICIT && lam != lam_last && lane == k - 1) r_d -= (lam_last - lam) * a_d;
         if (GRAMX && P.rconst != nullptr && lane < k) r_d += P.rconst[(size_t)d.row * P.ldr + lane];
@@ -1109,13 +1301,14 @@
         T p_d = r_d;
         T r_old = wave_sum(r_d * r_d);
         bool done = (r_old <= (T)1e-12);
-        for (int step = 0; step < P.max_cg_steps && !done; step++) {
-            T Ap_d = run_pass(p_d, std::integral_constant<int, 1>{});
+        for (int step = 0; step < P.max_cg_steps - (NEXT ? 1 : 0) && !done; step++) {
+            T Ap_d = run_pass(p_d, std::integral_constant<int, 1>{}, std::false_type{});
             Ap_d += lam * p_d;
             if (!IMPLICIT && lam != lam_last && lane == k - 1) Ap_d += (lam_last - lam) * p_d;
             if (lane >= k) Ap_d = T(0);
             T alpha = cg_div(r_old, wave_sum(Ap_d * p_d));
             a_d += alpha * p_d;
+            if (!NEXT && step == P.max_cg_steps - 1) break;
             r_d -= alpha * Ap_d;
             T r_new = wave_sum(r_d * r_d);
             if (r_new <= (T)1e-8) done = true;
@@ -1124,6 +1317,14 @@
                 r_old = r_new;
             }
         }
+        if (NEXT && P.max_cg_steps > 0 && !done) {
+            T Ap_d = run_pass(p_d, std::integral_constant<int, 1>{}, std::true_type{});
+            Ap_d += lam * p_d;
+            if (!IMPLICIT && lam != lam_last && lane == k - 1) Ap_d += (lam_last - lam) * p_d;
+            if (lane >= k) Ap_d = T(0);
+            const T alpha = cg_div(r_old, wave_sum(Ap_d * p_d));
+            a_d += alpha * p_d;
+        } else if constexpr (NEXT) gather_row(tile, dn, pn);
         if (lane < k) P.A[(size_t)d.row * P.lda + lane] = a_d;
     };
 
@@ -1145,10 +1346,12 @@
         Pre p0 = load_pre(d0);
         Tile tA;
         int pend = issue_claim();
+        if constexpr (EARLY) gather_row(tA, d0, p0);
         while (rix < P.nrows) {
             const bool shrt = short_row(d0.nnz);
             if (CMF_DBG(P, 1)) {
                 dbg_fill_tile<(NE == 2) ? 2 : 4, S>(tA, (T)(p0.idx & 3) * (T)0.001);
+            } else if constexpr (EARLY) {
             } else if constexpr (MIX) {
                 if (shrt) load_tile2<T, S>(tA, P.B, P.ldb, k, p0.idx, d0.nnz, lane);
                 else load_tile_ne(tA, P.B, P.ldb, k, p0.idx, d0.nnz, lane);
@@ -1156,9 +1359,9 @@
             RowDesc d2 = load_desc(rnn);
             Pre p1 = load_pre(d1);
             if constexpr (MIX) {
-                if (shrt) solve(d0, p0, tA, std::true_type{});
-                else solve(d0, p0, tA, std::false_type{});
-            } else solve(d0, p0, tA, std::false_type{});
+                if (shrt) solve(d0, p0, tA, std::true_type{}, std::true_type{}, d1, p1);
+                else solve(d0, p0, tA, std::false_type{}, std::true_type{}, d1, p1);
+            } else solve(d0, p0, tA, std::false_type{}, std::true_type{}, d1, p1);
             const int r3 = cbase + CG_NCOUNTERS * __builtin_amdgcn_readfirstlane(pend);
             d0 = d1; p0 = p1; d1 = d2;
             rix = rnxt; rnxt = rnn; rnn = r3;
@@ -1176,13 +1379,13 @@
         if (d1.nnz > 0) load_tile_ne(tB, P.B, P.ldb, k, p1.idx, d1.nnz, lane);
         RowDesc d3 = load_desc(rix + 3 * nwaves);
         Pre p2 = load_pre(d2);
-        solve(d0, p0, tA, std::false_type{});
+        solve(d0, p0, tA, std::false_type{}, std::false_type{}, d1, p1);
         rix += nwaves;
         if (rix >= P.nrows) break;
         if (d2.nnz > 0) load_tile_ne(tA, P.B, P.ldb, k, p2.idx, d2.nnz, lane);
         RowDesc d4 = load_desc(rix + 3 * nwaves);
         Pre p3 = load_pre(d3);
-        solve(d1, p1, tB, std::false_type{});
+        solve(d1, p1, tB, std::false_type{}, std::false_type{}, d2, p2);
         rix += nwaves;
         d0 = d2; p0 = p2; d1 = d3; p1 = p3; d2 = d4;
     }
diff --git a/cmfrec_amd/csrc/device.hpp b/cmfrec_amd/csrc/device.hpp
--- a/cmfrec_amd/csrc/device.hpp
+++ b/cmfrec_amd/csrc/device.hpp
@@ -424,6 +424,45 @@
     HIP_CHECK(hipGetLastError());
 }
 
+struct CappedDesc {
+    RowDesc *dev = nullptr;
+    int nrows = 0;
+    void build(const RowDesc *desc_dev, int count, int nteams, hipStream_t st)
+    {
+        std::vector<RowDesc> h((size_t)count);
+        HIP_CHECK(hipMemcpyAsync(h.data(), desc_dev, (size_t)count * sizeof(RowDesc), hipMemcpyDeviceToHost, st));
+        HIP_CHECK(hipStreamSynchronize(st));
+        const int per_round = nteams;
+        const int rest = count - nteams;
+        const int last = nteams + ((rest - 1) / per_round) * CG_NCOUNTERS + (rest - 1) % per_round;
+        nrows = last + 1;
+        RowDesc none; none.row = 0; none.nnz = 0; none.st = 0;
+        std::vector<RowDesc> out((size_t)nrows, none);
+        for (int i = 0; i < count; i++) {
+            const int pos = (i < nteams) ? i : nteams + ((i - nteams) / per_round) * CG_NCOUNTERS + (i - nteams) % per_round;
+            out[(size_t)pos] = h[(size_t)i];
+        }
+        HIP_CHECK(hipMalloc((void **)&dev, (size_t)nrows * sizeof(RowDesc)));
+        HIP_CHECK(hipMemcpyAsync(dev, out.data(), (size_t)nrows * sizeof(RowDesc), hipMemcpyHostToDevice, st));
+        HIP_CHECK(hipStreamSynchronize(st));
+    }
+    void release(hipStream_t st)
+    {
+        if (dev == nullptr) return;
+        HIP_CHECK(hipStreamSynchronize(st));
+        HIP_CHECK(hipFree(dev));
+        dev = nullptr;
+    }
+};
+inline bool cg_teams_cap(int &grid, int teams_per_block, int count)
+{
+    const int cap = switches().cg_teams;
+    if (cap <= 0) return false;
+    grid = std::min(grid, (cap + teams_per_block - 1) / teams_per_block);
+    const int nteams = grid * teams_per_block;
+    return nteams < CG_NCOUNTERS && nteams < count;
+}
+
 template <int S, bool IMPLICIT, int W, int RPB, bool GRAMX = false, int NRES_ = 0, int NTSEL = 0>
 inline void launch_cg_bin(const DeviceInfo &dev, CgParams<real_t> P, int first, int count, BinTimers *tm, int bin, hipStream_t st, int counter_set = -1)
 {
@@ -453,8 +492,15 @@
     }
     int teams_needed = (count + RPB - 1) / RPB;
     int grid = std::min(teams_needed, dev.num_cus * blocks_per_cu);
+    CappedDesc capped;
+    if (cg_teams_cap(grid, RPB, count)) {
+        capped.build(P.desc, count, grid * RPB, st);
+        P.desc = capped.dev;
+        P.nrows = capped.nrows;
+    }
     hipLaunchKernelGGL(kern, dim3(grid), dim3(threads), smem, st, P);
     HIP_CHECK(hipGetLastError());
+    capped.release(st);
     if (tm) {
         HIP_CHECK(hipEventRecord(ev.b, st));
         tm->ev[bin].push_back(ev);
@@ -491,8 +537,15 @@
             HIP_CHECK(hipOccupancyMaxActiveBlocksPerMultiprocessor(&nb, kern, 256, smem));
             blocks_per_cu = std::max(1, nb);
         }
-        const int grid = std::min((count + 3) / 4, dev.num_cus * blocks_per_cu);
+        int grid = std::min((count + 3) / 4, dev.num_cus * blocks_per_cu);
+        CappedDesc capped;
+        if (cg_teams_cap(grid, 4, count)) {
+            capped.build(P1.desc, count, grid * 4, st);
+            P1.desc = capped.dev;
+            P1.nrows = capped.nrows;
+        }
         hipLaunchKernelGGL(kern, dim3(grid), dim3(256), smem, st, P1);
+        capped.release(st);
     }
     HIP_CHECK(hipGetLastError());
     if (tm) {
diff --git a/cmfrec_amd/csrc/device_base.hpp b/cmfrec_amd/csrc/device_base.hpp
--- a/cmfrec_amd/csrc/device_base.hpp
+++ b/cmfrec_amd/csrc/device_base.hpp
@@ -60,6 +60,7 @@
     bool eig_jacobi = false;
     int debug_skip = 0;
     bool debug_ticks = false;
+    int cg_teams = 0;
     int newrows_block_rows = 0;
     void reload()
     {
@@ -85,6 +86,7 @@
         v = str("CMFREC_HIP_EIG"); eig_jacobi = v && strcmp(v, "jacobi") == 0;
         debug_skip = num("CMFREC_HIP_CG_SKIP", num("CMFREC_HIP_CHOL_SKIP", num("CMFREC_HIP_WAVE_SKIP", 0)));
         debug_ticks = str("CMFREC_HIP_GRAM_TICKS") != nullptr || str("CMFREC_HIP_CHOL_TICKS") != nullptr;
+        cg_teams = num("CMFREC_HIP_CG_TEAMS", 0);
         newrows_block_rows = num("CMFREC_HIP_NEWROWS_BLOCK_ROWS", 0);
     }
 };
diff --git a/cmfrec_amd/csrc/gram_cg_kernels.hpp b/cmfrec_amd/csrc/gram_cg_kernels.hpp
--- a/cmfrec_amd/csrc/gram_cg_kernels.hpp
+++ b/cmfrec_amd/csrc/gram_cg_kernels.hpp
@@ -410,15 +410,23 @@
             T p = r;
             T r_old = lanes::wave_sum(r * r);
             if (r_old > (T)1e-12) {
-                for (int step = 0; step < P.max_cg_steps; step++) {
+                bool done = false;
+                for (int step = 0; step < P.max_cg_steps - 1 && !done; step++) {
                     const T Mp = mul(p);
                     const T Ap = live ? Mp : T(0);
                     const T alpha = cg_div(r_old, lanes::wave_sum(Ap * p));
                     a += alpha * p; r -= alpha * Ap;
                     const T r_new = lanes::wave_sum(r * r);
-                    if (r_new <= (T)1e-8) break;
-                    p = p * cg_div(r_new, r_old) + r;
-                    r_old = r_new;
+                    if (r_new <= (T)1e-8) done = true;
+                    else {
+                        p = p * cg_div(r_new, r_old) + r;
+                        r_old = r_new;
+                    }
+                }
+                if (P.max_cg_steps > 0 && !done) {
+                    const T Mp = mul(p);
+                    const T Ap = live ? Mp : T(0);
+                    a += cg_div(r_old, lanes::wave_sum(Ap * p)) * p;
                 }
             }
             if (live) arow[lane] = a;
```
